# foolwood/SiamMask

Measured on AMD Instinct MI355X. Metric: frames/sec (255x255 search, 127x127 template), higher is better.
Workload: dtype f16

## Files before the change

siammask_amd/_lib.py:

```python
import ctypes
import os
import subprocess

import torch

_HERE = os.path.dirname(os.path.abspath(__file__))
LIB_PATH = os.environ.get("SMK_LIB") or os.path.join(_HERE, "libsiammask_hip.so")
CSRC = os.path.join(_HERE, "csrc")

DTYPE = {"f32": 0, "fp32": 0, "float32": 0, "f16": 1, "fp16": 1, "float16": 1, "half": 1,
         "f16x3": 2}
VARIANT = {"rpn": 0, "base": 1, "sharp": 2}
TRACK_BOX, TRACK_MASK, TRACK_NO_MASK_HEAD = 0, 1, 2

SYMBOLS = (
    "smk_version", "smk_last_error", "smk_create", "smk_destroy", "smk_set_weight",
    "smk_finalize_weights", "smk_template", "smk_track", "smk_refine", "smk_set_decode_params", "smk_decode", "smk_step", "smk_set_graph_mode", "smk_seq_status", "smk_seq_sync_check", "smk_set_result_ring", "smk_result_ring_cursor", "smk_set_pipeline", "smk_pipeline_join", "smk_pipeline_observe",
    "smk_debug_read", "smk_debug_seq_inject", "smk_tune", "smk_tune_get", "smk_profile", "smk_profile_dump", "smk_op_conv2d_ex", "smk_op_conv2d", "smk_op_dw_xcorr",
    "smk_op_maxpool3x3s2", "smk_op_conv_seq", "smk_host_conv2d_ex", "smk_host_plan_conv", "smk_host_plan_seq", "smk_bench_conv", "smk_packed_size", "smk_export_packed",
    "smk_import_packed", "smk_crop_resize", "smk_paste_mask", "smk_paste_labels", "smk_mask_rbox_workspace", "smk_mask_rbox",
    "smk_trk_state_bytes", "smk_trk_set", "smk_trk_plan", "smk_trk_advance", "smk_crop_resize_dev", "smk_paste_mask_dev",
    "smk_host_trk_plan", "smk_host_trk_advance",
)


class ConvGeom(ctypes.Structure):
    _fields_ = [(n, ctypes.c_int) for n in (
        "B", "Cin", "H", "W", "Cout", "k", "stride", "pad", "dil", "relu", "res_mode",
        "win", "ups", "Hl", "Wl", "org_y", "org_x", "pos_mul", "pos_add", "cin_off", "cin_len")]


class SeqOp(ctypes.Structure):
    _fields_ = [("g", ConvGeom), ("src", ctypes.c_int), ("res_src", ctypes.c_int), ("sync", ctypes.c_int),
                ("cfg", ctypes.c_int), ("kstag", ctypes.c_int), ("w_host", ctypes.c_void_p), ("b_host", ctypes.c_void_p),
                ("y_dev", ctypes.c_void_p)]


class TrkCfg(ctypes.Structure):
    _fields_ = [("context_amount", ctypes.c_double), ("lr", ctypes.c_double)] + [(n, ctypes.c_int) for n in (
        "exemplar_size", "instance_size", "total_stride", "base_size", "score_size", "mask_size")]


class SmkError(RuntimeError):
    code = 0


E_SEQ = -6


def build_library(force=False, verbose=False):
    if force:
        subprocess.check_call(["make", "-C", CSRC, "clean"], stdout=subprocess.DEVNULL)
    out = subprocess.run(["make", "-C", CSRC, "-j", "4"], stdout=subprocess.PIPE,
                         stderr=subprocess.STDOUT, universal_newlines=True)
    if verbose or out.returncode != 0:
        print(out.stdout)
    if out.returncode != 0:
        raise SmkError("building libsiammask_hip.so failed")
    return LIB_PATH


_lib = None


def lib():
    global _lib
    if _lib is not None:
        return _lib
    if not os.path.exists(LIB_PATH):
        raise SmkError(
            "%s is missing: the HIP extension has not been built (run `python -c 'import "
            "__graft_entry__ as g; g.build()'` or `make -C siammask_amd/csrc`). There is no "
            "CPU fallback." % LIB_PATH)
    L = ctypes.CDLL(LIB_PATH)
    vp, ci, fp = ctypes.c_void_p, ctypes.c_int, ctypes.c_void_p
    L.smk_version.restype = ci
    L.smk_last_error.restype = ctypes.c_char_p
    L.smk_create.argtypes = [ctypes.POINTER(vp), ci, ci, ci, ci]
    L.smk_destroy.argtypes = [vp]
    L.smk_set_weight.argtypes = [vp, ctypes.c_char_p, fp, ctypes.POINTER(ctypes.c_int64), ci]
    L.smk_finalize_weights.argtypes = [vp]
    L.smk_template.argtypes = [vp, fp, ci, vp]
    L.smk_track.argtypes = [vp, fp, ci, ci, fp, fp, fp, vp]
    L.smk_refine.argtypes = [vp, vp, ci, ci, fp, vp]
    L.smk_set_decode_params.argtypes = [vp, fp, ci, ci, ctypes.c_double, ctypes.c_double]
    L.smk_decode.argtypes = [vp, fp, fp, ci, fp, vp, fp, vp]
    L.smk_step.argtypes = [vp, fp, ci, ci, fp, fp, fp, fp, fp, fp, vp]
    L.smk_set_graph_mode.argtypes = [vp, ci]
    L.smk_debug_seq_inject.argtypes = [vp, ci]
    L.smk_set_result_ring.argtypes = [vp, vp, vp, ci, ci]
    L.smk_set_pipeline.argtypes = [vp, ci]
    L.smk_pipeline_join.argtypes = [vp, vp]
    L.smk_pipeline_observe.argtypes = [vp, vp]
    L.smk_result_ring_cursor.argtypes = [vp, ctypes.POINTER(ci), ci, vp]
    L.smk_seq_sync_check.argtypes = [vp, vp, ctypes.POINTER(ci)]
    L.smk_tune.argtypes = [ctypes.c_char_p, ci]
    L.smk_tune_get.argtypes = [ctypes.c_char_p, ctypes.POINTER(ci)]
    L.smk_profile.argtypes = [vp, ci]
    L.smk_profile_dump.argtypes = [vp, ctypes.c_char_p, ci]
    ip = ctypes.POINTER(ci)
    L.smk_debug_read.argtypes = [vp, ctypes.c_char_p, fp, ip, ip, ip, vp]
    gp = ctypes.POINTER(ConvGeom)
    L.smk_op_conv2d_ex.argtypes = [ci, ci, gp, fp, fp, fp, fp, vp, fp, vp]
    L.smk_op_conv2d.argtypes = [ci, ci, fp, ci, ci, ci, ci, fp, fp, ci, ci, ci, ci, ci, ci, fp, fp, vp]
    L.smk_op_dw_xcorr.argtypes = [ci, fp, fp, ci, ci, ci, ci, ci, ci, fp, vp]
    L.smk_op_maxpool3x3s2.argtypes = [ci, fp, ci, ci, ci, ci, fp, vp]
    L.smk_host_conv2d_ex.argtypes = [gp, fp, fp, fp, fp, vp, fp]
    L.smk_host_plan_conv.argtypes = [gp, ci, ci, ip, ip, ip, ip]
    L.smk_packed_size.argtypes = [vp, ctypes.POINTER(ctypes.c_uint64)]
    L.smk_export_packed.argtypes = [vp, vp, ctypes.c_uint64]
    L.smk_import_packed.argtypes = [vp, vp, ctypes.c_uint64]
    L.smk_crop_resize.argtypes = [vp, ctypes.c_int64, ci, ci, vp, vp, ci, ci, fp, vp]
    L.smk_paste_mask.argtypes = [fp, ci, vp, ci, ci, ci, ctypes.c_float, ctypes.c_float, vp, fp, vp]
    L.smk_paste_labels.argtypes = [fp, ci, vp, ci, ci, ci, ctypes.c_float, ctypes.c_float, vp, vp]
    L.smk_mask_rbox_workspace.argtypes = [ci, ci, ci]
    L.smk_mask_rbox.argtypes = [vp, ci, ci, ci, ctypes.c_double, vp, ctypes.c_size_t, vp, vp]
    cp = ctypes.POINTER(TrkCfg)
    L.smk_trk_state_bytes.argtypes = [ci]
    L.smk_trk_set.argtypes = [vp, ci, vp, vp, vp, ci, ci, vp]
    L.smk_trk_plan.argtypes = [vp, ci, cp, vp]
    L.smk_trk_advance.argtypes = [vp, ci, cp, vp, ci, vp, ci, vp]
    L.smk_host_trk_plan.argtypes = [vp, ci, cp]
    L.smk_host_trk_advance.argtypes = [vp, ci, cp, vp, ci, vp, ci]
    L.smk_crop_resize_dev.argtypes = [vp, ctypes.c_int64, ci, ci, vp, ci, ci, fp, vp]
    L.smk_paste_mask_dev.argtypes = [fp, fp, ci, ci, vp, ci, ci, ci, ci, ctypes.c_float, ctypes.c_float, vp, fp, vp]
    L.smk_op_conv_seq.argtypes = [ctypes.POINTER(SeqOp), ci, fp, ci, ctypes.POINTER(ctypes.c_float), fp, ip, vp]
    L.smk_host_plan_seq.argtypes = [ctypes.POINTER(SeqOp), ci, ci, ip, ip, ip]
    L.smk_bench_conv.argtypes = [ci, ci, gp, ci, ci, ctypes.POINTER(ctypes.c_float), vp]
    for name in SYMBOLS:
        fn = getattr(L, name)
        if name not in ("smk_last_error",):
            fn.restype = ctypes.c_size_t if name in ("smk_mask_rbox_workspace", "smk_trk_state_bytes") else ci
    _lib = L
    for kv in filter(None, os.environ.get("SMK_TUNE", "").split(",")):
        k, v = kv.split("=")
        check(L.smk_tune(k.strip().encode(), int(v)))
    return L


def check(rc):
    if rc != 0:
        msg = lib().smk_last_error()
        e = SmkError("libsiammask_hip error %d: %s" % (rc, msg.decode() if msg else "?"))
        e.code = rc
        raise e


def current_stream_ptr():
    return ctypes.c_void_p(torch.cuda.current_stream().cuda_stream)


def tune(**kw):
    for k, v in kw.items():
        check(lib().smk_tune(k.encode(), int(v)))


def tune_get(key):
    v = ctypes.c_int(0)
    check(lib().smk_tune_get(key.encode(), ctypes.byref(v)))
    return v.value
```

siammask_amd/csrc/conv_igemm.hip:

```cpp
#include <hip/hip_runtime.h>
#include "smk_kernels.h"

namespace smk {

typedef _Float16 half8 __attribute__((ext_vector_type(8)));
typedef _Float16 half4 __attribute__((ext_vector_type(4)));
typedef float floatx16 __attribute__((ext_vector_type(16)));
typedef float floatx4 __attribute__((ext_vector_type(4)));

template <typename T> struct Traits;
template <> struct Traits<float> {
    static constexpr int VE = 4;
    typedef floatx4 frag_t;
    typedef floatx4 out4_t;
    static __device__ inline void mma(floatx16 &acc, const frag_t &a, const frag_t &b) {
        acc = __builtin_amdgcn_mfma_f32_32x32x2f32(a[0], b[0], acc, 0, 0, 0);
        acc = __builtin_amdgcn_mfma_f32_32x32x2f32(a[1], b[1], acc, 0, 0, 0);
        acc = __builtin_amdgcn_mfma_f32_32x32x2f32(a[2], b[2], acc, 0, 0, 0);
        acc = __builtin_amdgcn_mfma_f32_32x32x2f32(a[3], b[3], acc, 0, 0, 0);
    }
    static __device__ inline floatx4 load4(const float *p) { return *(const floatx4 *)p; }
    static __device__ inline void store4(float *p, floatx4 v) { *(floatx4 *)p = v; }
    static constexpr int EV = 4;
    static __device__ inline void loadv(const float *p, float (&v)[4]) {
// ... 760 lines not shown
        for (int q = 0; q < EV; q += 4) {
            const floatx4 b4 = *(const floatx4 *)(bias + n + q);
            bv[q] = b4[0]; bv[q + 1] = b4[1]; bv[q + 2] = b4[2]; bv[q + 3] = b4[3];
        }
        T *out = (T *)p.out;
        const float *ecol = ebase + ((c4 >> 6) * WK) * (64 * LDE) + (c4 & 63);
#pragma unroll
        for (int ps = 0; ps < NPASS; ++ps) {
            const int row = ps * RPP + r0;
            if (row < nvalid) {
                const float *er = ecol + ((row >> 6) * WN * WK) * (64 * LDE) + (row & 63) * LDE;
                float v[EV];
#pragma unroll
                for (int q = 0; q < EV; q += 4) {
                    floatx4 x = *(const floatx4 *)(er + q);
#pragma unroll
                    for (int kq = 1; kq < WK; ++kq) x += *(const floatx4 *)(er + kq * (64 * LDE) + q);
                    v[q] = x[0]; v[q + 1] = x[1]; v[q + 2] = x[2]; v[q + 3] = x[3];
                }
#pragma unroll
                for (int q = 0; q < EV; ++q) {
                    float x = v[q] + bv[q];
                    if (p.res_mode == RES_PRE_RELU) x += rv[ps][q];
                    if (p.relu) x = fmaxf(x, 0.f);
                    if (p.res_mode == RES_POST_RELU) x += rv[ps][q];
                    v[q] = x;
                }
                TR::storev(out + (size_t)(m0 + row) * p.Cos + p.cout_off + n, v);
            }
        }
    }
}

static int halo_patch_rows(const ConvParams &p, int BM) {
    const int howo = p.Ho * p.Wo, Wp = p.Wl + 2 * p.pad;
    const int tpi = (howo + BM - 1) / BM;
    int worst = 0;
    for (int tl = 0; tl < tpi; ++tl) {
        const int ml0 = tl * BM, nv = howo - ml0 < BM ? howo - ml0 : BM;
        const int oy0 = ml0 / p.Wo, ox0 = ml0 % p.Wo, ml = ml0 + nv - 1, oyl = ml / p.Wo, oxl = ml % p.Wo;
        const int rows = oyl * Wp + oxl - (oy0 * Wp + ox0) + 2 * p.dil * Wp + 2 * p.dil + 1;
        if (rows > worst) worst = rows;
    }
    return worst;
}
constexpr int HALO_AROWS_128 = 320, HALO_AROWS_64 = 224;

template <typename T, int WM, int WN, int WK, int AROWS, int NSLOT, int NPATCH>
static int launch_halo_t(const ConvParams &p, hipStream_t s) {
    constexpr int BM = 64 * WM, BN = 64 * WN;
    const int tpi = (p.Ho * p.Wo + BM - 1) / BM;
    if (halo_patch_rows(p, BM) > AROWS) return 1;
    dim3 grid(p.B * tpi * ((p.Nst + BN - 1) / BN));
    hipLaunchKernelGGL((conv3x3_halo_kernel<T, WM, WN, WK, AROWS, NSLOT, NPATCH>), grid, dim3(512), 0, s, p);
    return hipGetLastError() == hipSuccess ? 0 : -4;
}

bool conv_halo_eligible(const ConvParams &p, int dtype, int bm) {
    const int ch = dtype == DT_F16 ? 64 : 32;
    if (p.kh != 3 || p.kw != 3 || p.stride != 1 || p.stride_x != 1 || p.ups || p.groups > 1 || p.Ci % ch != 0 ||
        p.out_mode != OUT_NHWC || !p.buf_lds || p.Wo != p.Wl + 2 * p.pad - 2 * p.dil)
        return false;
    return halo_patch_rows(p, bm == 128 ? 128 : 64) <= (bm == 128 ? HALO_AROWS_128 : HALO_AROWS_64);
}

int launch_conv_halo(const ConvParams &p, int dtype, int bm, void *stream) {
    hipStream_t s = (hipStream_t)stream;
    const int ch = dtype == DT_F16 ? 64 : 32;
    if (!conv_halo_eligible(p, dtype, bm)) return 1;
    const int ch_n = p.Ci / ch;
    const long wgs64 = (long)p.B * ((p.Ho * p.Wo + 63) / 64) * ((p.Nst + 127) / 128);
    const bool db = bm == 64 && g_tune.halo_db && ch_n >= 2 && wgs64 <= 256;
    if (dtype == DT_F16) {
        if (bm == 128) return launch_halo_t<_Float16, 2, 2, 1, HALO_AROWS_128, 2, 1>(p, s);
        return db ? launch_halo_t<_Float16, 1, 2, 2, HALO_AROWS_64, 3, 2>(p, s) : launch_halo_t<_Float16, 1, 2, 2, HALO_AROWS_64, 3, 1>(p, s);
    }
    if (bm == 128) return launch_halo_t<float, 2, 2, 1, HALO_AROWS_128, 2, 1>(p, s);
    return db ? launch_halo_t<float, 1, 2, 2, HALO_AROWS_64, 3, 2>(p, s) : launch_halo_t<float, 1, 2, 2, HALO_AROWS_64, 3, 1>(p, s);
}

}
namespace smk {
#include "refine_chain_body.inc"
constexpr int CM_CONV_LDS = IgemmLds<2, 2, 1, 128, 2>::v;
constexpr int CM_LDS = CMax<RC_LDS, 2 * CM_CONV_LDS>::v;

__global__ __launch_bounds__(1024) void chain_mask_kernel(const RefineChainParams rp, const ConvBatch cb) {
    __shared__ __attribute__((aligned(16))) unsigned char smem[CM_LDS];
    if ((int)blockIdx.x < rp.B) {
        refine_chain_body<false>(rp, (int)blockIdx.x, smem);
    } else {
        const int half = threadIdx.x >> 9;
        const int bx = 2 * ((int)blockIdx.x - rp.B) + half;
        if (bx < cb.start[cb.n])
            conv_igemm_body<_Float16, 2, 2, 1, 128, OUT_NCHW_F32, 2>(cb, bx, 0, half * 512, smem + half * CM_CONV_LDS);
    }
    if (rp.tail_sem) {
        __syncthreads();
        if (threadIdx.x == 0) {
            const unsigned prev = __hip_atomic_fetch_add(rp.tail_sem + 5, 1u, __ATOMIC_RELAXED, __HIP_MEMORY_SCOPE_AGENT);
            if (prev == gridDim.x - 1) {
                __hip_atomic_store(rp.tail_sem + 5, 0u, __ATOMIC_RELAXED, __HIP_MEMORY_SCOPE_AGENT);
                __hip_atomic_fetch_add(rp.tail_sem, 1u, __ATOMIC_RELEASE, __HIP_MEMORY_SCOPE_AGENT);
            }
        }
    }
}

int launch_chain_mask(const RefineChainParams &rp, ConvBatch &cb, void *stream) {
    if (rp.v2_cs != 32 || rp.v1_cs != 16 || rp.v0_cs != 8 || cb.n != 1) return -1;
    ConvParams &p = cb.p[0];
    if (p.out_mode != OUT_NCHW_F32 || p.groups > 1) return -1;
    const int tiles = ((p.M + 127) / 128) * ((p.Nst + 127) / 128);
    if (tiles & 1) return 1;
    cb.start[0] = 0;
    for (int i = 1; i <= CONV_BATCH_MAX; ++i) cb.start[i] = tiles;
    p.ksplit = 1;
    hipLaunchKernelGGL(chain_mask_kernel, dim3(rp.B + (tiles + 1) / 2), dim3(1024), 0, (hipStream_t)stream, rp, cb);
    return hipGetLastError() == hipSuccess ? 0 : -4;
}

template <typename T>
__global__ void conv_naive_kernel(const ConvParams p) {
    typedef Traits<T> TR;
    constexpr int VE = TR::VE;
    const int g = blockIdx.z;
    const int cin_off = p.cin_off + g * p.g_cin_off;
    const T *wgt = (const T *)p.wgt + (size_t)g * p.g_wgt_off * p.Kpad;
    const float *bias = p.bias + g * p.g_wgt_off;
    const int cout_off = p.cout_off + g * p.g_cout_off;
    const int nq = p.Nst / 4;
    const long total = (long)p.M * nq;
    const T *in = (const T *)p.in;
    for (long idx = (long)blockIdx.x * blockDim.x + threadIdx.x; idx < total;
         idx += (long)gridDim.x * blockDim.x) {
        const int m = (int)(idx / nq), n = (int)(idx - (long)m * nq) * 4;
        const RowInfo r = row_info(p, m, p.pos);
        float acc[4] = {0.f, 0.f, 0.f, 0.f};
        for (int kvec = 0; kvec < p.K; kvec += VE) {
            const KDecode d = decode_k(kvec, p.Ci, p.kw);
            const long off = gather_offset(p, r, d, cin_off);
            if (off < 0) continue;
            for (int e = 0; e < VE; ++e) {
                const float a = (float)in[off + e];
                for (int j = 0; j < 4; ++j)
                    acc[j] = fmaf(a, (float)wgt[(size_t)(n + j) * p.Kpad + kvec + e], acc[j]);
            }
        }
        if (p.out_mode == OUT_NHWC) {
            floatx4 v = {acc[0] + bias[n], acc[1] + bias[n + 1], acc[2] + bias[n + 2], acc[3] + bias[n + 3]};
            floatx4 rv = {0.f, 0.f, 0.f, 0.f};
            if (p.res_mode != RES_NONE)
                rv = TR::load4((const T *)p.res + (size_t)m * p.res_Cs + p.res_coff + n);
            if (p.res_mode == RES_PRE_RELU) v += rv;
            if (p.relu)
                for (int j = 0; j < 4; ++j) v[j] = fmaxf(v[j], 0.f);
            if (p.res_mode == RES_POST_RELU) v += rv;
            TR::store4((T *)p.out + (size_t)m * p.Cos + cout_off + n, v);
        } else {
            const int hw = p.Ho * p.Wo;
            const int b = m / hw, pos = m - b * hw;
            for (int j = 0; j < 4; ++j)
                if (n + j < p.N) {
                    float v = acc[j] + bias[n + j];
                    if (p.relu) v = fmaxf(v, 0.f);
                    ((float *)p.out)[((size_t)b * p.N + n + j) * hw + pos] = v;
                }
        }
    }
}

Tuning g_tune;

static int default_kt(int bm, int bn) { return (bm == 64 && bn == 64) ? 256 : 128; }
static int default_stages(int bm, int bn, int kt) {
    if (bm == 128 && bn == 128 && kt == 128) return 2;
    return (bm + bn) * kt * 3 <= 160 * 1024 ? 3 : 2;
}

TileChoice choose_tile(const ConvParams &p, int dtype) {
    (void)dtype;
    TileChoice t;
    if (g_tune.force_tile) {
        static const int tb[6][2] = {{0, 0}, {128, 128}, {128, 64}, {64, 128}, {64, 64}, {256, 128}};
        t.bm = tb[g_tune.force_tile][0];
        t.bn = tb[g_tune.force_tile][1];
        t.stages = default_stages(t.bm, t.bn, default_kt(t.bm, t.bn));
    } else {
        const long ng = p.groups > 0 ? p.groups : 1;
        auto tiles = [&](int bm, int bn) {
            return (long)((p.M + bm - 1) / bm) * ((p.Nst + bn - 1) / bn) * ng * 16 / g_tune.min_blocks_x16;
        };
        if (p.Nst <= 64) {
            if (tiles(128, 64) >= 200) { t.bm = 128; t.bn = 64; t.stages = 3; }
            else { t.bm = 64; t.bn = 64; t.stages = 3; }
        } else if (tiles(256, 128) >= 900 && p.K >= 2048) { t.bm = 256; t.bn = 128; t.stages = 3; }
        else if (tiles(128, 128) >= 300) { t.bm = 128; t.bn = 128; t.stages = 2; }
        else if (tiles(64, 128) >= 200) { t.bm = 64; t.bn = 128; t.stages = 3; }
        else { t.bm = 64; t.bn = 64; t.stages = 3; }
    }
    t.kt = g_tune.kt ? g_tune.kt : default_kt(t.bm, t.bn);
// ... 117 lines not shown
```

siammask_amd/csrc/conv_plan.cpp:

```cpp
#include "conv_plan.h"

#include <algorithm>
#include <cstdio>
#include <cstdlib>
#include <cstring>

using namespace smk;

TileChoice tile_from_code(int code, const ConvParams &p, int dtype) {
    TileChoice t = choose_tile(p, dtype);
    static const int tb[6][2] = {{0, 0}, {128, 128}, {128, 64}, {64, 128}, {64, 64}, {256, 128}};
    const int tile = code & 15, kt = (code >> 4) & 3, st = (code >> 6) & 3;
    if (tile >= 1 && tile <= 5) {
        t.bm = tb[tile][0]; t.bn = tb[tile][1];
        t.kt = (t.bm == 64 && t.bn == 64) ? 256 : 128;
        t.stages = (t.bm == 128 && t.bn == 128) ? 2 : 3;
    }
    if (kt) t.kt = kt == 2 ? 256 : 128;
    if (t.bm == 64 && t.bn == 64) t.kt = 256;
    if (t.bm == 256) t.kt = 128;
    if (st) t.stages = st + 1;
    return t;
}

// ... 252 lines not shown
    return st;
}

double seq_fabric_bytes(const SeqLayer *L, int n, int B, const void *late_read) {
    double ext = 0.0;
    for (int i = 0; i < n; ++i) {
        const SeqLayer &l = L[i];
        bool in_inside = false, res_inside = l.res == nullptr, out_read = false;
        for (int j = 0; j < n; ++j) {
            if (j < i && L[j].out == l.in) in_inside = true;
            if (j < i && l.res && L[j].out == l.res) res_inside = true;
            if (j > i && (L[j].in == l.out || L[j].res == l.out)) out_read = true;
        }
        bool in_counted = false, res_counted = false;
        for (int j = 0; j < i; ++j) {
            if (L[j].in == l.in || L[j].res == l.in) in_counted = true;
            if (l.res && (L[j].in == l.res || L[j].res == l.res)) res_counted = true;
        }
        const double px_in = (double)B * l.Hs * l.Ws, px_out = (double)B * l.Ho * l.Wo;
        ext += (double)l.Nst * l.Kpad * 2.0;
        if (!in_inside && !in_counted) ext += px_in * l.Cs * 2.0;
        if (!res_inside && !res_counted) ext += px_out * l.res_Cs * 2.0;
        if (!out_read || l.out == late_read) ext += px_out * l.Nst * 2.0;
    }
    return ext;
}

const int WREG_TILE[9][2] = {{0, 0}, {64, 256}, {64, 128}, {64, 64}, {128, 256}, {128, 128}, {128, 64}, {96, 256}, {32, 64}};
int wreg_choice(const ConvParams &p, const ConvOpt &o, int dtype, long ncu) {
    if (o.algo_naive || !conv_wreg_eligible(p, dtype)) return 0;
    if (o.wreg) return o.wreg;
    if (g_tune.wreg >= 2) return g_tune.wreg - 1;
    if (!g_tune.wreg) return 0;
    const long K = (long)p.kh * p.kw * p.Ci;
    if (g_tune.wreg_policy == 1) {
        if (p.kh > 3) return 0;
        if (p.kh == 3 && p.stride == 1 && K <= 1152) return 0;
        if (p.M > 16384 && !(p.Nst >= 512 || (K >= 2304 && p.Nst >= 128) || (K >= 1024 && p.Nst >= 256) ||
                             (p.kh == 3 && p.stride == 2)))
            return 0;
        static const int cand[4] = {4, 1, 2, 3};
        const int nr = (p.Nst + 63) / 64 * 64, ng = p.groups > 0 ? p.groups : 1;
        for (int ci = 0; ci < 4; ++ci) {
            const int bm = WREG_TILE[cand[ci]][0], bn = WREG_TILE[cand[ci]][1];
            if (bn > nr && bn > 64) continue;
            if ((long)((p.M + bm - 1) / bm) * ((p.Nst + bn - 1) / bn) * ng >= 150) {
                if (cand[ci] == 4 && g_tune.wreg96) {
                    const long tn = (p.Nst + 255) / 256 * ng;
                    const long t128 = (long)((p.M + 127) / 128) * tn, t96 = (long)((p.M + 95) / 96) * tn;
                    if (((t128 + ncu - 1) / ncu) * 128 > ((t96 + ncu - 1) / ncu) * 96 && t96 <= 4 * ncu) return 7;
                }
                return cand[ci];
            }
        }
        if (g_tune.wreg32 && (long)((p.M + 63) / 64) * ((p.Nst + 63) / 64) * ng < g_tune.wreg32) return 8;
        return 3;
    }
    if (p.M < 4096) return 0;
    if (p.kh == 3 && K >= 2304 && p.Nst >= 512)
        return ((long)((p.M + 127) / 128) * ((p.Nst + 255) / 256) >= 200) ? 4 : 1;
    if (p.M > 16384) return 0;
    if (p.kh == 1 && K >= 512 && p.Nst <= 256) return p.Nst >= 192 ? 2 : 3;
    if (p.kh == 3 && p.stride == 2 && K >= 1152 && p.Nst <= 128) return 3;
    return 0;
}
int wreg_stages(int ctx_dtype, int B) {
    if (g_tune.wreg_stages) return g_tune.wreg_stages;
    return (ctx_dtype == DT_F16X3 || (B >= 1 && B <= 2)) ? 4 : 3;
}
int wreg_stages_from_code(int code) {
    const int st = (code >> 6) & 3;
    return st == 0 ? wreg_stages(DT_F16, 0) : (st == 1 ? 8 : (st == 2 ? 3 : 4));
}

bool pp_choice(const ConvParams &p, const ConvOpt &o, int dtype, long ncu) {
    if (!g_tune.pp || o.algo_naive || o.halo || o.wreg || o.tile_code || !conv_pp_eligible(p, dtype)) return false;
    const long K = (long)p.kh * p.kw * p.Ci;
    const long tiles = (long)((p.M + 255) / 256) * ((p.Nst + 255) / 256);
    const long rounds = (tiles + ncu - 1) / ncu;
    if (tiles < 200 || tiles * 10 < rounds * ncu * 9 || p.Nst < 256 || (p.Nst % 256) != 0) return false;
    return g_tune.pp == 2 || K >= 2304;
}

ConvPlan plan_conv(const ConvParams &p, const ConvOpt &o, const PackedConv &pc, int dtype, int B, long ncu) {
    const int kd = kdtype(dtype);
    ConvPlan pl;
    pl.tile = tile_from_code(o.tile_code, p, kd);
    if (o.algo_naive) { pl.kind = CK_NAIVE; return pl; }
    int bm = halo_choice(pc, p, o, kd);
    if (bm && !o.halo && conv_ksplit(p, kd, pl.tile) > 1) bm = 0;
    if (pp_choice(p, o, kd, ncu)) { pl.kind = CK_PP; return pl; }
    const int wr = (o.halo || (bm && !o.wreg && g_tune.wreg < 2 && g_tune.wreg_policy == 0)) ? 0 : wreg_choice(p, o, kd, ncu);
    if (wr) {
        pl.kind = CK_WREG; pl.wreg = wr; pl.stages = wreg_stages(dtype, B);
    } else if (bm && conv_halo_eligible(p, kd, bm)) {
        pl.kind = CK_HALO; pl.halo_bm = bm;
    }
    return pl;
}

ConvPlan plan_conv_batch(const ConvBatch &cb, const ConvOpt *const o[], int lead, int dtype, int B, long ncu) {
    const int kd = kdtype(dtype);
    ConvPlan pl;
    int wr = wreg_choice(cb.p[lead], *o[lead], kd, ncu);
    for (int i = 0; i < cb.n && wr; ++i)
        if (!wreg_choice(cb.p[i], *o[i], kd, ncu) || (cb.p[i].groups > 1) != (cb.p[0].groups > 1)) wr = 0;
    if (wr) {
        pl.kind = CK_WREG; pl.wreg = wr; pl.stages = wreg_stages(dtype, B);
    } else {
        pl.tile = tile_from_code(o[lead]->tile_code, cb.p[lead], kd);
    }
    return pl;
}

std::string plan_kernel_name(const ConvPlan &pl, int dtype, int out_mode, int merged) {
    const char *dt = dtname(kdtype(dtype));
    char kn[80], mg[16] = "";
    if (merged) snprintf(mg, sizeof(mg), ",merged%d", merged);
    switch (pl.kind) {
    case CK_NAIVE: return "conv_naive";
    case CK_PP: return "conv_pp<f16,256x256>";
    case CK_HALO: snprintf(kn, sizeof(kn), "conv3x3_halo<%s,%dx128>", dt, pl.halo_bm); break;
    case CK_WREG: snprintf(kn, sizeof(kn), "conv_wreg<%s,%dx%d,s%d%s>", dt, WREG_TILE[pl.wreg][0], WREG_TILE[pl.wreg][1], pl.stages, mg); break;
    default:
        snprintf(kn, sizeof(kn), "conv_igemm<%s,%dx%dx%d,s%d,%s%s>", dt, pl.tile.bm, pl.tile.bn, pl.tile.kt, pl.tile.stages,
                 out_mode == OUT_NCHW_F32 ? "nchw" : "nhwc", mg);
    }
    return kn;
}
```

siammask_amd/csrc/conv_plan.h:

```cpp
#pragma once
#include <string>
#include <vector>

#include "smk_kernels.h"

struct Act {
    void *p = nullptr;
    int H = 0, W = 0, C = 0;
};

struct PackedConv {
    void *w = nullptr;
    void *w_halo = nullptr;
    void *w_frag = nullptr;
    void *w_frag_halo = nullptr;
    void *w_frag16 = nullptr;
    float *bias = nullptr;
    int N = 0;
    int rows = 0;
    int group_rows = 0;
    int groups = 1;
    int Ci = 0, k = 1, K = 0, Kpad = 0;
    int kw = 0;
    int alg_k = 0;
    float *oscale = nullptr;
    int x3_ct = 0, x3_nreal = 0;
    bool x3 = false;
};

struct ConvOpt {
    int stride = 1, pad = 0, dil = 1, relu = 0;
    int stride_x = 0;
    const Act *res = nullptr;
    int res_mode = smk::RES_NONE;
    int res_coff = 0;
    int cin_off = 0;
    int cout_off = 0;
    int n_override = 0;
    int groups = 1;
    bool win = false;
    int Hl = 0, Wl = 0, org_y = 0, org_x = 0;
    const int *pos = nullptr;
    int pos_mul = 0, pos_add = 0;
    bool ups = false;
    float *nchw_out = nullptr;
    int algo_naive = 0;
    int tile_code = 0;
    int halo = 0;
    int wreg = 0;
};

inline int kdtype(int dtype) { return dtype == smk::DT_F16X3 ? smk::DT_F16 : dtype; }
inline const char *dtname(int dt) { return dt == smk::DT_F16 ? "f16" : "f32"; }

#pragma GCC visibility push(hidden)

enum ConvKernel { CK_NAIVE, CK_IGEMM, CK_HALO, CK_WREG, CK_PP };
struct ConvPlan {
    int kind = CK_IGEMM;
    smk::TileChoice tile{};
    int halo_bm = 0;
    int wreg = 0;
    int stages = 0;
};

extern const int WREG_TILE[9][2];

smk::TileChoice tile_from_code(int code, const smk::ConvParams &p, int dtype);
int halo_choice(const PackedConv &pc, const smk::ConvParams &p, const ConvOpt &o, int dtype);
int wreg_choice(const smk::ConvParams &p, const ConvOpt &o, int dtype, long ncu);
int wreg_stages(int ctx_dtype, int B);
int wreg_stages_from_code(int code);
bool pp_choice(const smk::ConvParams &p, const ConvOpt &o, int dtype, long ncu);

ConvPlan plan_conv(const smk::ConvParams &p, const ConvOpt &o, const PackedConv &pc, int dtype, int B, long ncu);
ConvPlan plan_conv_batch(const smk::ConvBatch &cb, const ConvOpt *const *o, int lead, int dtype, int B, long ncu);
std::string plan_kernel_name(const ConvPlan &pl, int dtype, int out_mode, int merged = 0);

bool seq_halo_ok(const smk::ConvParams &p, int bm);
bool seq_layer_from(const smk::ConvParams &p, int dtype, smk::SeqLayer &L, int force_halo = 0);
bool seq_pair_fusable(const smk::SeqLayer *L, int i, int *code);
bool seq_pair_fits(const smk::SeqLayer *L, int i, int B, int *code);

struct SeqRec {
    smk::SeqLayer L;
    const void *wstd = nullptr;
    std::string id;
};
struct SeqPlanEnv {
    int B = 0;
    int nslots = 0;
    bool have_xch = false;
};
struct SeqPlanStats { int pairs = 0, triples = 0, resident = 0; };

SeqPlanStats plan_seq(std::vector<SeqRec> &rec, const SeqPlanEnv &env, const char *locked, const std::vector<const void *> &read_after);
double seq_fabric_bytes(const smk::SeqLayer *L, int n, int B, const void *late_read);

#pragma GCC visibility pop
```

siammask_amd/csrc/engine.cpp:

```cpp
#include <hip/hip_runtime_api.h>

#include <cmath>
#include <cstdarg>
#include <tuple>
#include <cstdio>
#include <cstdlib>
#include <cstring>
#include <functional>
#include <map>
#include <set>
#include <memory>
#include <string>
#include <vector>

#include "../../include/siammask_hip.h"
#include "../../include/siammask_hip_test.h"
#include "conv_plan.h"
#include "smk_kernels.h"
#include "tracker_state.h"

using namespace smk;

static thread_local std::string g_err;
static int g_concurrency_default = 0;
// ... 171 lines not shown
    const char *p3_buf = "a";
    bool graph_mode = false;
    hipStream_t cap_stream = nullptr;
    std::map<GraphKey, hipGraphExec_t> graphs;
    std::map<GraphKey, unsigned long long> graph_used;
    unsigned long long graph_tick = 0;

    std::map<std::string, PackedConv> conv;
    std::map<std::string, void *> buf;
    std::map<std::string, size_t> buf_elems;
    std::set<std::string> buf_alias;
    int *pos_dev = nullptr;
    void *dec_scratch = nullptr;
    float *ks_part = nullptr;
    unsigned *ks_cnt = nullptr;
    unsigned *seq_bar = nullptr;
    float *seq_xch = nullptr;
    int *seq_err = nullptr;
    int *seq_err_host = nullptr;
    int *seq_err_hdev = nullptr;
    int seq_fail = 0;
    bool seq_pending = false;
    std::map<GraphKey, bool> graph_has_seq;
    unsigned long long *seq_clk = nullptr, *seq_clk2 = nullptr;
    int seq_grid = 0;
    bool seq_on = false;
    struct SeqList {
        std::vector<SeqRec> rec;
        double flop = 0.0, bytes = 0.0;
        void clear() { rec.clear(); flop = bytes = 0.0; }
    } seq;

    double *ring_box = nullptr;
    void *ring_ref = nullptr;
    int ring_rows = 0;
    int *ring_cursor = nullptr;

    float anchor_w[8] = {104, 88, 64, 40, 32}, anchor_h[8] = {32, 40, 64, 80, 96};
    int anchor_stride = 8;
    double *window_dev = nullptr;
    double penalty_k = 0.04, window_influence = 0.4;

    bool concurrency = true;
    hipStream_t side[2] = {nullptr, nullptr};
    std::vector<hipEvent_t> ev_pool;
    size_t ev_next = 0;

    bool prof = false;
    bool prof_merge = false;
    struct ProfRec { std::string id, kernel; double flop, bytes; hipEvent_t e0, e1; double ext_bytes = 0.0; };
    std::vector<ProfRec> prof_recs;
    std::vector<hipEvent_t> prof_pool;
    size_t prof_pool_next = 0;

    int pipe_depth = 0;
    int parity_now = 0;
    int pipe_parity = 0;
    int last_parity = 0;
    hipStream_t pipe_stream = nullptr;
    std::vector<hipEvent_t> pipe_ev;
    size_t pipe_ev_next = 0;
    bool tail_pending = false;
    hipEvent_t tail_ev = nullptr;
    int ring_batch = 0;
    unsigned *pipe_cnt = nullptr;
    bool tail2_pending = false;
    GraphKey tail2_key, tail2_gated_key;
    int wave_prio_now = 0;
};

struct StepRec {
    bool gate_late = false;
    bool mark_fold = false;
    bool two = false;
    bool seq_exit = false;
    bool tail_fold = false;
    bool defer_mask = false;
    bool ring = false;
    bool ring_refine = false;
    bool seq_exit_done = false;
    bool done_folded = false;
    bool ring_ref_folded = false;
    bool has_seq = false;
    bool mask_join_pending = false;
    struct DeferredMask {
        bool have = false;
        ConvParams p = {};
        double flop = 0.0, bytes = 0.0;
    } deferred_mask;
};

struct ProfScope {
    smk_ctx *c; hipStream_t s; int idx = -1;
    ProfScope(smk_ctx *c_, hipStream_t s_, const std::string &id, const std::string &kernel, double flop,
              double bytes) : c(c_), s(s_) {
        if (!c->prof) return;
        smk_ctx::ProfRec r{id, kernel, flop, bytes, nullptr, nullptr, 0.0};
        if (c->prof_pool_next + 2 > c->prof_pool.size()) return;
        r.e0 = c->prof_pool[c->prof_pool_next++];
        r.e1 = c->prof_pool[c->prof_pool_next++];
        (void)hipEventRecord(r.e0, s);
        c->prof_recs.push_back(r);
        idx = (int)c->prof_recs.size() - 1;
    }
    ~ProfScope() { if (idx >= 0) (void)hipEventRecord(c->prof_recs[idx].e1, s); }
    void ext_bytes(double b) { if (idx >= 0) c->prof_recs[idx].ext_bytes = b; }
    void cancel() { if (idx >= 0 && idx == (int)c->prof_recs.size() - 1) { c->prof_recs.pop_back(); c->prof_pool_next -= 2; } idx = -1; }
};

static int stream_dep(smk_ctx *c, hipStream_t from, hipStream_t to) {
    hipEvent_t e = c->ev_pool[c->ev_next++ % c->ev_pool.size()];
    HIPCHK(hipEventRecord(e, from));
    HIPCHK(hipStreamWaitEvent(to, e, 0));
    return 0;
}
static bool parallel_ok(const smk_ctx *c) { return c->concurrency && !c->prof && c->side[0] && c->side[1]; }

static int nbranch(const smk_ctx *c) { return c->variant == SMK_VARIANT_RPN ? 2 : 3; }

static const HostTensor *find_w(const smk_ctx *c, const std::string &name) {
    auto it = c->host_w.find(name);
    return it == c->host_w.end() ? nullptr : &it->second;
}

static int fold(const smk_ctx *c, const ConvPart &part, int Cout, std::vector<double> &scale,
                std::vector<double> &shift) {
    scale.assign(Cout, 1.0);
    shift.assign(Cout, 0.0);
    if (!part.bn.empty()) {
        const HostTensor *g = find_w(c, part.bn + ".weight"), *b = find_w(c, part.bn + ".bias");
        const HostTensor *m = find_w(c, part.bn + ".running_mean"), *v = find_w(c, part.bn + ".running_var");
        if (!g || !b || !m || !v) return fail(SMK_E_WEIGHT, "missing BatchNorm tensors for %s", part.bn.c_str());
        if ((int)g->data.size() != Cout || (int)b->data.size() != Cout || (int)m->data.size() != Cout ||
            (int)v->data.size() != Cout)
            return fail(SMK_E_WEIGHT, "BatchNorm %s has wrong size", part.bn.c_str());
        for (int i = 0; i < Cout; ++i) {
            const double inv = (double)g->data[i] / std::sqrt((double)v->data[i] + 1e-5);
            scale[i] = inv;
            shift[i] = (double)b->data[i] - (double)m->data[i] * inv;
        }
    }
    if (!part.bias.empty()) {
        const HostTensor *b = find_w(c, part.bias);
        if (!b || (int)b->data.size() != Cout) return fail(SMK_E_WEIGHT, "missing/mis-sized %s", part.bias.c_str());
        for (int i = 0; i < Cout; ++i) shift[i] += (double)b->data[i];
    }
    return 0;
}

static void split_rows_x3(std::vector<float> &rows, int nrows, int Kpad1, int Kpad3, int taps, int Ci0, std::vector<float> &oscale) {
    std::vector<float> out((size_t)nrows * Kpad3, 0.f);
    oscale.assign(nrows, 1.f);
    for (int n = 0; n < nrows; ++n) {
        float mx = 0.f;
        for (int k = 0; k < taps * Ci0; ++k) mx = std::max(mx, std::fabs(rows[(size_t)n * Kpad1 + k]));
        int e = 0;
        if (mx > 0.f) {
            e = 13 - (int)std::floor(std::log2(mx));
            e = std::max(-8, std::min(e, 40));
        }
        const float sc = std::ldexp(1.f, e);
        oscale[n] = std::ldexp(1.f, -e);
        for (int t = 0; t < taps; ++t)
            for (int ci = 0; ci < Ci0; ++ci) {
                const float v = rows[(size_t)n * Kpad1 + (size_t)t * Ci0 + ci] * sc;
                const float hi = (float)(_Float16)v, lo = (float)(_Float16)(v - hi);
                float *d = out.data() + (size_t)n * Kpad3 + (size_t)t * 3 * Ci0 + ci;
                d[0] = hi; d[Ci0] = lo; d[2 * Ci0] = hi;
            }
// ... 477 lines not shown
        snprintf(idn, sizeof(idn), "seq[%s..%s]", r[0].id.c_str(), r[a.n - 1].id.c_str());
        const double fr = (double)a.n / (double)n;
        ProfScope ps(c, s, idn, "conv_seq", c->seq.flop * fr, c->seq.bytes * fr);
        ps.ext_bytes(seq_fabric_bytes(a.L, a.n, B, buf("p2")));
        if (launch_conv_seq(a, c->seq_grid, s))
            return fail(SMK_E_HIP, "launch of %s failed: %s", idn, hipGetErrorString(hipGetLastError()));
        c->seq_pending = rec.has_seq = true;
        if (want_clk) {
            unsigned long long h[2 * SEQ_MAX + 1], h2[(12 + 32) * SEQ_MAX];
            HIPCHK(hipStreamSynchronize(s));
            HIPCHK(hipMemcpy(h, c->seq_clk, sizeof(h), hipMemcpyDeviceToHost));
            if (want_clk2) HIPCHK(hipMemcpy(h2, c->seq_clk2, sizeof(h2), hipMemcpyDeviceToHost));
            seq_print_clk(a, r, idn, h, want_clk2 ? h2 : nullptr);
        }
    }
    c->seq.clear();
    return 0;
}

static int seq_health(smk_ctx *c) {
    if (!c->seq_err_host) return 0;
    const int e = *(volatile int *)c->seq_err_host;
    if (!e) return 0;
    (void)hipDeviceSynchronize();
    c->seq_fail = e;
    if (e != 3) c->seq_grid = 0;
    else c->pipe_depth = 0;
    if (c->pipe_cnt) {
        const unsigned init[16] = {1u, 0u};
        (void)hipMemcpy(c->pipe_cnt, init, sizeof(init), hipMemcpyHostToDevice);
    }
    *(volatile int *)c->seq_err_host = 0;
    (void)hipMemset(c->seq_err, 0, sizeof(int));
    (void)hipMemset(c->seq_bar, 0, 8 * 32 * sizeof(unsigned));
    for (auto &kv : c->graphs) hipGraphExecDestroy(kv.second);
    c->graphs.clear();
    c->graph_used.clear();
    c->graph_has_seq.clear();
    c->seq_pending = false;
    c->tail_pending = false;
    c->tail2_pending = false;
    c->template_B = 0;
    c->track_B = 0;
    if (e == 3)
        return fail(SMK_E_SEQ, "conv_seq_kernel reported: (pipelined step) a gate waited 0.2 s (a tail's gate: 5 s) for its partner on the other stream -- something serialises "
                    "the two queues of this context (a profiler collecting counters does); the results of the calls enqueued on this context "
                    "since then are invalid (the cached template included) and frame steps are serial from here on: call template() again and "
                    "re-submit the frame");
    return fail(SMK_E_SEQ, "conv_seq_kernel reported %s: the results of the calls enqueued on this context since then are invalid "
                "(the cached template included); persistent sequences are now off for this context (per-layer kernels from here "
                "on): call template() again and re-submit the frame",
                e == 1 ? "an uneven distribution of workgroups over the XCDs" : "a team-barrier time-out (another kernel held CUs "
                "for more than 0.2 s, or a second persistent kernel ran beside it)");
}

static bool seq_wanted(const smk_ctx *c, int B) {
    if (!g_tune.seq || c->seq_grid <= 0 || c->dtype != DT_F16) return false;
    if (B >= g_tune.seq_min_batch && B <= g_tune.seq_max_batch) return true;
    if (B == g_tune.seq_extra_batch) return true;
    return B % 8 == 0 && B <= g_tune.seq_mult_max;
}

static void conv_work(const PackedConv &pc, const ConvParams &p, int B, int dtype, double &flop, double &bytes) {
    const int ng = p.groups > 0 ? p.groups : 1;
    const double kreal = pc.alg_k ? (double)pc.alg_k : (double)p.kh * p.kw * p.Ci;
    const size_t es = esize(kdtype(dtype));
    flop += 2.0 * p.M * (double)p.N * kreal * ng;
    bytes += (double)B * (p.ups ? p.Hs * p.Ws : (double)p.Hl * p.Wl) * p.Ci * es * ng + (double)p.M * p.N * ng * (p.out_mode == OUT_NCHW_F32 ? 4 : es) +
             (double)p.N * kreal * es * ng + (p.res ? (double)p.M * p.N * es : 0.0);
}

static int launch_plan(const ConvPlan &pl, ConvBatch &cb, const void *w_halo, int dtype, hipStream_t s, const char *what) {
    int rc;
    switch (pl.kind) {
    case CK_PP: rc = launch_conv_pp(cb.p[0], s); break;
    case CK_WREG: rc = launch_conv_wreg_batch(cb, WREG_TILE[pl.wreg][0], WREG_TILE[pl.wreg][1], pl.stages, s); break;
    case CK_HALO: {
        ConvParams ph = cb.p[0];
        ph.wgt = w_halo;
        rc = launch_conv_halo(ph, dtype, pl.halo_bm, s);
        break;
    }
    case CK_NAIVE: rc = launch_conv_naive(cb.p[0], dtype, s); break;
    default: rc = launch_conv_mfma_batch(cb, dtype, pl.tile, s);
    }
    if (rc == 1) return fail(SMK_E_STATE, "internal: %s is not eligible for the kernel planned for it", what);
    if (rc) return fail(SMK_E_HIP, "launch of %s failed: %s", what, hipGetErrorString(hipGetLastError()));
    return 0;
}

static int run_conv(smk_ctx *c, const char *id, const Act &in, const Act *out, int B, const ConvOpt &o,
                    hipStream_t s, StepRec *rec = nullptr) {
    auto it = c->conv.find(id);
    if (it == c->conv.end()) return fail(SMK_E_STATE, "internal: conv %s not packed", id);
    ConvBatch cb;
    cb.n = 1;
    ConvParams &p = cb.p[0];
    CHK(conv_params(conv_env(c), it->second, in, out, B, o, p));
    double flop = 0.0, bytes = 0.0;
    conv_work(it->second, p, B, c->dtype, flop, bytes);
    if (c->seq_on) {
        SeqLayer L;
        if (!o.algo_naive && !o.halo && !o.wreg && !o.tile_code && seq_layer_from(p, kdtype(c->dtype), L)) {
            c->seq.rec.push_back({L, p.wgt_frag, id});
            c->seq.flop += flop;
            c->seq.bytes += bytes;
            return 0;
        }
        if (!rec) return fail(SMK_E_STATE, "internal: conv %s recorded into a sequence without a step record", id);
        CHK(seq_flush(c, *rec, B, s));
    }
    const ConvPlan pl = plan_conv(p, o, it->second, c->dtype, B, c->ncu);
    ProfScope ps(c, s, id, plan_kernel_name(pl, c->dtype, p.out_mode), flop, bytes);
    char what[80];
    snprintf(what, sizeof(what), "conv %s", id);
    return launch_plan(pl, cb, it->second.w_halo, kdtype(c->dtype), s, what);
}

struct ConvJob { const char *id; const Act *in; const Act *out; ConvOpt o; };

static int run_conv_jobs(smk_ctx *c, const std::vector<ConvJob> &jobs, int B, int lead, hipStream_t s, StepRec *rec = nullptr) {
    if (jobs.empty() || (int)jobs.size() > CONV_BATCH_MAX) return fail(SMK_E_ARG, "internal: bad conv job count");
    if (c->seq_on) {
        const size_t n0 = c->seq.rec.size();
        for (auto &j : jobs) CHK(run_conv(c, j.id, *j.in, j.out, B, j.o, s, rec));
        if (c->seq.rec.size() == n0 + jobs.size())
            for (size_t i = n0; i + 1 < c->seq.rec.size(); ++i) c->seq.rec[i].L.sync = 0;
        return 0;
    }
    ConvBatch cb;
    cb.n = (int)jobs.size();
    bool split_for_halo = g_tune.halo != 0;
    int n_halo = 0;
    for (int i = 0; i < cb.n; ++i) {
        auto it = c->conv.find(jobs[i].id);
        if (it == c->conv.end()) return fail(SMK_E_STATE, "internal: conv %s not packed", jobs[i].id);
        CHK(conv_params(conv_env(c), it->second, *jobs[i].in, jobs[i].out, B, jobs[i].o, cb.p[i]));
        const int bm = halo_choice(it->second, cb.p[i], jobs[i].o, kdtype(c->dtype));
        if (bm) ++n_halo;
        if (bm == 64 || (bm == 0 && cb.p[i].kh == 3)) split_for_halo = false;
    }
    const bool merge_ok = g_tune.merge && (g_tune.merge == 2 || B <= g_tune.merge_max_batch);
    if ((c->prof && !c->prof_merge) || cb.n == 1 || !merge_ok || (split_for_halo && n_halo)) {
        for (auto &j : jobs) CHK(run_conv(c, j.id, *j.in, j.out, B, j.o, s));
        return 0;
    }
    double mflop = 0.0, mbytes = 0.0;
    std::string mid;
    const ConvOpt *opts[CONV_BATCH_MAX];
    for (int i = 0; i < cb.n; ++i) {
        opts[i] = &jobs[i].o;
        if (!c->prof) continue;
        conv_work(c->conv.find(jobs[i].id)->second, cb.p[i], B, c->dtype, mflop, mbytes);
        mid += (i ? "+" : "") + std::string(jobs[i].id);
    }
    const ConvPlan pl = plan_conv_batch(cb, opts, lead, c->dtype, B, c->ncu);
    ProfScope ps(c, s, mid.c_str(), plan_kernel_name(pl, c->dtype, cb.p[lead].out_mode, cb.n), mflop, mbytes);
    char what[80];
    snprintf(what, sizeof(what), "merged conv %s..", jobs[0].id);
    return launch_plan(pl, cb, nullptr, kdtype(c->dtype), s, what);
}

static int run_conv_pair(smk_ctx *c, const char *id3, const Act &in3, const Act &out3, const ConvOpt &o3, const char *id1,
                         const Act &out1, const ConvOpt &o1, int B, hipStream_t s) {
    if (c->dtype != DT_F16 || !g_tune.pair_launch || c->seq_on || parallel_ok(c) || (c->prof && !c->prof_merge)) return 1;
    if (g_tune.pair_launch == 1 && B < 3) return 1;
// ... 137 lines not shown
            if (b == 0) {
                Act r = act(c, RN[st], so, so, X(planes * 4));
                ConvOpt od;
                if (st == 0) { od.stride = 1; od.pad = 0; }
                else if (st == 1) { od.stride = 2; od.pad = 0; }
                else { od.stride = 1; od.pad = 1; }
                if (par) {
                    hipStream_t sd = c->side[0];
                    CHK(stream_dep(c, s, sd));
                    CHK(run_conv(c, id_ds.c_str(), cur, &r, B, od, sd, &rec));
                    CHK(run_conv(c, id_c1.c_str(), cur, &t1, B, o1, s, &rec));
                } else {
                    CHK(run_conv_jobs(c, {{id_ds.c_str(), &cur, &r, od}, {id_c1.c_str(), &cur, &t1, o1}}, B, 0, s, &rec));
                }
                res = r;
            } else if (!c1_done) {
                CHK(run_conv(c, id_c1.c_str(), cur, &t1, B, o1, s, &rec));
            }
            c1_done = false;
            CHK(run_conv(c, (id + "c2").c_str(), t1, &t2, B, o2, s, &rec));
            if (b == 0 && par) CHK(stream_dep(c, c->side[0], s));
            const bool last = b == STAGE_BLOCKS[st] - 1;
            const char *oname = last ? (st == 0 ? "p1" : st == 1 ? "p2" : AN[2]) : ((b & 1) ? BN[st] : AN[st]);
            if (last && st == 2 && cur.p == c->buf.at(AN[2])) oname = BN[2];
            Act out = act(c, oname, so, so, X(planes * 4));
            if (last && st == 2) c->p3_buf = oname;
            ConvOpt o3; o3.relu = 1; o3.res = &res; o3.res_mode = RES_PRE_RELU;
            int paired = 1;
            if (!c->seq_on && st >= 1) {
                if (!last) {
                    char idn[32];
                    snprintf(idn, sizeof(idn), "l%d.%d.c1", st + 1, b + 1);
                    Act t1n = act(c, T1N[st], so, so, X(planes));
                    ConvOpt o1n; o1n.relu = 1;
                    paired = run_conv_pair(c, (id + "c3").c_str(), t2, out, o3, idn, t1n, o1n, B, s);
                    if (paired < 0) return paired;
                    if (paired == 0) c1_done = true;
                } else if (st == 2 && so >= 20) {
                    Act se = act(c, "search", so, so, X(256));
                    ConvOpt oa0;
                    paired = run_conv_pair(c, (id + "c3").c_str(), t2, out, o3, "adjust", se, oa0, B, s);
                    if (paired < 0) return paired;
                    if (paired == 0) adjust_done = true;
                }
            }
            if (paired == 1) CHK(run_conv(c, (id + "c3").c_str(), t2, &out, B, o3, s, &rec));
            cur = out;
            sp = so;
        }
    }
    ConvOpt oa;
    if (sp < 20) {
        Act zf = act(c, "zf", sp - 8, sp - 8, X(256));
        oa.win = true; oa.Hl = oa.Wl = sp - 8; oa.org_y = oa.org_x = 4;
        CHK(run_conv(c, "adjust", cur, &zf, B, oa, s, &rec));
    } else if (!adjust_done) {
        Act se = act(c, "search", sp, sp, X(256));
        CHK(run_conv(c, "adjust", cur, &se, B, oa, s, &rec));
    }
    if (c->seq_on && search_nb > 0 && sp >= 20 && g_tune.seq_search && c->seq.rec.size() < (size_t)SEQ_MAX) {
        Act se = act(c, "search", sp, sp, X(256));
        Act xs = act(c, "xs", sp - 2, sp - 2, X(256 * search_nbt));
        ConvOpt o; o.relu = 1; o.n_override = 256 * search_nb;
        CHK(run_conv(c, "conv_search", se, &xs, B, o, s, &rec));
        if (search_done) *search_done = true;
    }
    if (c->seq_on) CHK(seq_flush(c, rec, B, s));
    c->last_B = B; c->last_S = S;
    return 0;
}

static int seq_template(smk_ctx *c, StepRec &rec, const float *z, int B, hipStream_t s) {
    auto X = [c](int C) { return c->dtype == DT_F16X3 ? X3_PLANES * C : C; };
    CHK(run_backbone(c, rec, z, B, 127, s));
    const int nb = nbranch(c);
    Act zf = act(c, "zf", 7, 7, X(256));
    Act zk = act(c, "zk", 5, 5, X(256 * nb));
    ConvOpt o; o.relu = 1;
    CHK(run_conv(c, "conv_kernel", zf, &zk, B, o, s));
    return 0;
}

static int seq_track(smk_ctx *c, StepRec &rec, const float *x, int B, int flags, float *cls, float *loc, float *mask,
                     hipStream_t s, bool defer_mask_join = false, int phase = PH_ALL) {
    auto X = [c](int C) { return c->dtype == DT_F16X3 ? X3_PLANES * C : C; };
    const bool x3 = c->dtype == DT_F16X3;
    const int nbt = nbranch(c);
    const int nb = (flags & SMK_TRACK_MASK) ? nbt : 2;
    bool search_done = false;
    CHK(run_backbone(c, rec, x, B, 255, s, phase, nb, nbt, &search_done));
    Act se = act(c, "search", 31, 31, X(256));
    Act xs = act(c, "xs", 29, 29, X(256 * nbt));
    ConvOpt o; o.relu = 1; o.n_override = 256 * nb;
    if (!search_done) CHK(run_conv(c, "conv_search", se, &xs, B, o, s));
    if (rec.gate_late) {
        if (launch_pipe_gate(c->pipe_cnt, c->seq_err, c->seq_err_hdev, s, 0, nullptr, c->pipe_cnt + 8)) return fail(SMK_E_HIP, "pipe_gate launch failed");
        rec.has_seq = true;
    }
    Act corr = act(c, "corr", 25, 25, X(256 * nbt));
    Act h0 = act(c, "head0", 25, 25, X(256 * nbt));
    const bool par = parallel_ok(c);
    const bool want_mask = (flags & SMK_TRACK_MASK) && !(flags & SMK_TRACK_NO_MASK_HEAD);
    hipStream_t s_loc = par ? c->side[0] : s, s_cls = (par && want_mask) ? c->side[1] : s;
    bool fused_heads = false;
    if (c->dtype == DT_F16 && g_tune.corr_head && !par) {
        auto ih = c->conv.find("head0"), ic = c->conv.find("cls3"), il = c->conv.find("loc3");
        if (ih != c->conv.end() && ic != c->conv.end() && il != c->conv.end() && ih->second.w_frag && ic->second.w_frag && il->second.w_frag &&
            ih->second.Kpad == 256 && ic->second.Kpad == 256 && il->second.Kpad == 256 && ih->second.group_rows == 256 &&
            ic->second.N == 10 && il->second.N == 20) {
            CorrHeadParams hp;
            memset(&hp, 0, sizeof(hp));
            hp.xs = (const _Float16 *)xs.p; hp.zk = (const _Float16 *)c->buf.at("zk"); hp.corr = (_Float16 *)corr.p; hp.h0 = (_Float16 *)h0.p;
            hp.w0_frag = ih->second.w_frag; hp.b0 = ih->second.bias; hp.w0_bytes = (unsigned)((size_t)ih->second.rows * ih->second.Kpad * 2);
            hp.w3_frag[0] = ic->second.w_frag; hp.b3[0] = ic->second.bias; hp.out3[0] = cls; hp.n3[0] = 10;
            hp.w3_frag[1] = il->second.w_frag; hp.b3[1] = il->second.bias; hp.out3[1] = loc; hp.n3[1] = 20;
            hp.w3_bytes[0] = (unsigned)((size_t)ic->second.rows * ic->second.Kpad * 2);
            hp.w3_bytes[1] = (unsigned)((size_t)il->second.rows * il->second.Kpad * 2);
            hp.B = B; hp.nb = nb; hp.Cs = 256 * nbt;
            const double flop = 2.0 * B * nb * 256.0 * 625 * 25 + 2.0 * B * nb * 625.0 * 256 * 256 + 2.0 * B * 625.0 * 256 * 30;
            const double bytes = (double)B * nb * 256.0 * (29 * 29 + 25 + 2 * 625) * 2 + 3.0 * 256 * 256 * 2 + (double)B * 30 * 625 * 4;
            ProfScope ps(c, s, "dw_xcorr+head0+cls3+loc3", "corr_head", flop, bytes);
            if (launch_corr_head(hp, s)) return fail(SMK_E_HIP, "corr_head launch failed: %s", hipGetErrorString(hipGetLastError()));
            fused_heads = true;
        }
    }
    if (!fused_heads) {
    XcorrParams xp{xs.p, c->buf.at("zk"), corr.p, B, 29, 29, 5, 5, 25, 25, 256 * nb, 256 * nbt};
    {
        const double xb = (double)B * nb * 256.0 * (29 * 29 + 25 + 625) * esize(c->dtype);
        ProfScope ps(c, s, "dw_xcorr", x3 ? "dw_xcorr_x3" : "dw_xcorr", 2.0 * B * nb * 256.0 * 625 * 25, x3 ? (double)X3_PLANES * xb : xb);
        if (x3 ? launch_xcorr_x3(xp, s) : launch_xcorr(xp, kdtype(c->dtype), s)) return fail(SMK_E_HIP, "xcorr launch failed");
    }
    ConvOpt oh; oh.relu = 1; oh.groups = nb;
    CHK(run_conv(c, "head0", corr, &h0, B, oh, s));
    if (par) { CHK(stream_dep(c, s, s_loc)); if (s_cls != s) CHK(stream_dep(c, s, s_cls)); }
    ConvOpt oc; oc.nchw_out = cls; oc.cin_off = 0;
    ConvOpt ol; ol.nchw_out = loc; ol.cin_off = x3 ? X3_PLANES * 256 : 256;
    if (par) {
        CHK(run_conv(c, "cls3", h0, nullptr, B, oc, s_cls));
        CHK(run_conv(c, "loc3", h0, nullptr, B, ol, s_loc));
    } else {
        CHK(run_conv_jobs(c, {{"cls3", &h0, nullptr, oc}, {"loc3", &h0, nullptr, ol}}, B, 1, s));
    }
    }
    if (want_mask) {
        ConvOpt om; om.nchw_out = mask; om.cin_off = x3 ? 2 * X3_PLANES * 256 : 512;
        if (rec.defer_mask && !par) {
            auto it = c->conv.find("mask3");
            if (it == c->conv.end()) return fail(SMK_E_STATE, "internal: conv mask3 not packed");
            CHK(conv_params(conv_env(c), it->second, h0, nullptr, B, om, rec.deferred_mask.p));
            const ConvParams &mp = rec.deferred_mask.p;
            rec.deferred_mask.flop = 2.0 * mp.M * (double)mp.N * mp.kh * mp.kw * mp.Ci;
            rec.deferred_mask.bytes = (double)mp.M * mp.Ci * esize(c->dtype) + (double)mp.M * mp.N * 4 + (double)mp.N * mp.Ci * esize(c->dtype);
            rec.deferred_mask.have = true;
        } else if (defer_mask_join && !par && !c->prof && g_tune.mask_overlap && c->side[0]) {
            CHK(stream_dep(c, s, c->side[0]));
            CHK(run_conv(c, "mask3", h0, nullptr, B, om, c->side[0]));
            rec.mask_join_pending = true;
        } else {
            CHK(run_conv(c, "mask3", h0, nullptr, B, om, s));
        }
    }
    if (par) { CHK(stream_dep(c, s_loc, s)); if (s_cls != s) CHK(stream_dep(c, s_cls, s)); }
    c->last_nb = nb;
    return 0;
}

static bool refine_splittable(const smk_ctx *c, int B) {
    return kdtype(c->dtype) == DT_F16 && g_tune.chain && !parallel_ok(c) && g_tune.merge && (g_tune.merge == 2 || B <= g_tune.merge_max_batch);
}
static int seq_refine(smk_ctx *c, StepRec &rec, int B, float *out, hipStream_t s, int part = 0) {
    const int *pos = c->pos_dev;
    auto X = [c](int C) { return c->dtype == DT_F16X3 ? X3_PLANES * C : C; };
    Act corr = act(c, "corr", 25, 25, X(256 * 3));
    Act p0 = act(c, "p0", 125, 125, X(64)), p1 = act(c, "p1", 63, 63, X(256)), p2 = act(c, "p2", 31, 31, X(512));
    ConvOpt r3; r3.pad = 1; r3.relu = 1;
    ConvOpt w2 = r3; w2.win = true; w2.Hl = w2.Wl = 15; w2.pos = pos; w2.pos_mul = 1; w2.pos_add = -4;
    ConvOpt w1 = r3; w1.win = true; w1.Hl = w1.Wl = 31; w1.pos = pos; w1.pos_mul = 2; w1.pos_add = -8;
    ConvOpt w0 = r3; w0.win = true; w0.Hl = w0.Wl = 61; w0.pos = pos; w0.pos_mul = 4; w0.pos_add = -16;
    const bool par = parallel_ok(c);
    hipEvent_t ev_v2 = nullptr, ev_v1 = nullptr, ev_v0 = nullptr;
    if (par) {
        hipStream_t sd = c->side[0];
        CHK(stream_dep(c, s, sd));
        Act v2a_ = act(c, "rf_v2a", 15, 15, 128), v1a_ = act(c, "rf_v1a", 31, 31, 64), v0a_ = act(c, "rf_v0a", 61, 61, 16);
        CHK(run_conv(c, "v2.0", p2, &v2a_, B, w2, sd));
        ev_v2 = c->ev_pool[c->ev_next++ % c->ev_pool.size()];
        HIPCHK(hipEventRecord(ev_v2, sd));
        CHK(run_conv(c, "v1.0", p1, &v1a_, B, w1, sd));
        ev_v1 = c->ev_pool[c->ev_next++ % c->ev_pool.size()];
        HIPCHK(hipEventRecord(ev_v1, sd));
        CHK(run_conv(c, "v0.0", p0, &v0a_, B, w0, sd));
        ev_v0 = c->ev_pool[c->ev_next++ % c->ev_pool.size()];
        HIPCHK(hipEventRecord(ev_v0, sd));
    }
    Act d1 = act(c, "rf_d", 1, 1, 15 * 15 * 32);
    ConvOpt od; od.win = true; od.Hl = od.Wl = 1; od.pos = pos; od.pos_mul = 1; od.cin_off = c->dtype == DT_F16X3 ? 2 * X3_PLANES * 256 : 512;
    Act v2a = act(c, "rf_v2a", 15, 15, 128), v1a = act(c, "rf_v1a", 31, 31, 64), v0a = act(c, "rf_v0a", 61, 61, 16);
    const bool merged = !par && (!c->prof || c->prof_merge) && g_tune.merge && (g_tune.merge == 2 || B <= g_tune.merge_max_batch);
    if (merged && part != 2) {
        w2.tile_code = 4;
        if (g_tune.rf_wreg & 1) w2.wreg = w1.wreg = w0.wreg = od.wreg = ((g_tune.rf_wreg >> 4) & 15) ? ((g_tune.rf_wreg >> 4) & 15) : 3;
        CHK(run_conv_jobs(c, {{"v2.0", &p2, &v2a, w2}, {"v1.0", &p1, &v1a, w1}, {"v0.0", &p0, &v0a, w0},
                              {"deconv", &corr, &d1, od}}, B, 0, s));
    } else if (part != 2) {
        CHK(run_conv(c, "deconv", corr, &d1, B, od, s));
    }
    Act d = act(c, "rf_d", 15, 15, 32);
    if (kdtype(c->dtype) == DT_F16 && g_tune.chain && !par) {
        if (!merged && part != 2) {
            CHK(run_conv(c, "v2.0", p2, &v2a, B, w2, s));
            CHK(run_conv(c, "v1.0", p1, &v1a, B, w1, s));
            CHK(run_conv(c, "v0.0", p0, &v0a, B, w0, s));
        }
        Act V2 = act(c, "rf_s2", 15, 15, 32), V1 = act(c, "rf_s1", 31, 31, 16), V0 = act(c, "rf_s0", 61, 61, 8);
        ConvOpt r3l = r3;
        r3l.tile_code = g_tune.rf_tile2;
        ConvOpt r3w = r3;
        if ((g_tune.rf_wreg & 2) && merged) r3l.wreg = r3w.wreg = ((g_tune.rf_wreg >> 8) & 15) ? ((g_tune.rf_wreg >> 8) & 15) : 3;
        if (part != 2) CHK(run_conv_jobs(c, {{"v2.2", &v2a, &V2, r3l}, {"v1.2", &v1a, &V1, r3w}, {"v0.2", &v0a, &V0, r3w}}, B, 0, s));
        if (part == 1) return 0;
        static const char *ids[9] = {"h2.0", "h2.2", "post0", "h1.0", "h1.2", "post1", "h0.0", "h0.2", "post2"};
        static const int geo[9][3] = {{225, 32, 32}, {225, 32, 32}, {961, 32, 16}, {961, 16, 16}, {961, 16, 16},
                                      {3721, 16, 4}, {3721, 4, 4}, {3721, 4, 4}, {16129, 4, 1}};
        RefineChainParams rp;
        double flop = 0.0, wbytes = 0.0;
        for (int i = 0; i < 9; ++i) {
            auto it = c->conv.find(ids[i]);
            if (it == c->conv.end()) return fail(SMK_E_STATE, "internal: conv %s not packed", ids[i]);
            const PackedConv &pc = it->second;
            if (pc.k != 3 || pc.groups != 1 || pc.Ci < geo[i][1] || pc.N != geo[i][2])
                return fail(SMK_E_STATE, "internal: conv %s does not have the Refine geometry", ids[i]);
            rp.L[i] = RefineChainLayer{pc.w, pc.bias, pc.Kpad, pc.Ci};
            flop += 2.0 * B * geo[i][0] * 9.0 * geo[i][1] * geo[i][2];
            wbytes += 2.0 * 9.0 * geo[i][1] * geo[i][2];
        }
        rp.d = d.p;
        rp.v2 = V2.p; rp.v1 = V1.p; rp.v0 = V0.p;
        rp.v2_cs = V2.C; rp.v1_cs = V1.C; rp.v0_cs = V0.C;
        rp.out = out;
        rp.B = B;
        rp.clk = nullptr;
        rp.ring = nullptr; rp.ring_cursor = nullptr; rp.ring_done = nullptr; rp.ring_rows = 0;
        rp.tail_sem = nullptr;
        if (rec.ring && c->ring_ref) {
            rp.ring = (_Float16 *)c->ring_ref; rp.ring_cursor = c->ring_cursor; rp.ring_done = (unsigned *)(c->ring_cursor + 1);
            rp.ring_rows = c->ring_rows;
            rec.ring_ref_folded = true;
        }
        static const bool want_clk = getenv("SMK_CHAIN_CLK") != nullptr;
        static unsigned long long *clk_dev = nullptr;
        hipStreamCaptureStatus cst = hipStreamCaptureStatusNone;
        if (want_clk && hipStreamIsCapturing(s, &cst) == hipSuccess && cst == hipStreamCaptureStatusNone) {
            if (!clk_dev) HIPCHK(hipMalloc((void **)&clk_dev, 32 * sizeof(unsigned long long)));
            rp.clk = clk_dev;
        }
        const double cbytes = B * (2.0 * (7200 + 225 * 32 + 961 * 16 + 3721 * 4) + 4.0 * 16129) + wbytes;
        if (rec.deferred_mask.have && !rp.clk) {
            ConvBatch cb;
            cb.n = 1;
            cb.p[0] = rec.deferred_mask.p;
            ProfScope ps(c, s, "refine_chain+mask3", "chain_mask", flop + rec.deferred_mask.flop, cbytes + rec.deferred_mask.bytes);
            if (rec.tail_fold) rp.tail_sem = c->pipe_cnt;
            const int rc = launch_chain_mask(rp, cb, s);
            rp.tail_sem = nullptr;
            if (rc == 0) {
                rec.deferred_mask.have = false;
                if (rec.tail_fold) rec.done_folded = true;
                return 0;
            }
            if (rc != 1) return fail(SMK_E_HIP, "chain_mask launch failed: %s", hipGetErrorString(hipGetLastError()));
            ps.cancel();
        }
        ProfScope ps(c, s, "refine_chain", "refine_chain", flop, cbytes);
        if (launch_refine_chain(rp, s)) return fail(SMK_E_HIP, "refine_chain launch failed: %s", hipGetErrorString(hipGetLastError()));
        if (rp.clk) {
            unsigned long long hh[22];
            HIPCHK(hipStreamSynchronize(s));
            HIPCHK(hipMemcpy(hh, clk_dev, sizeof(hh), hipMemcpyDeviceToHost));
            {
                const unsigned long long *h = hh;
                fprintf(stderr, "refine_chain layers (us): load=%.2f", (double)(h[1] - h[0]) * 0.01);
                for (int i = 0; i < 9; ++i) fprintf(stderr, " %s=%.2f", ids[i], (double)(h[i + 2] - h[i + 1]) * 0.01);
                fprintf(stderr, " total=%.2f\n", (double)(h[10] - h[0]) * 0.01);
            }
        }
        return 0;
    }
    Act h2a = act(c, "rf_h2a", 15, 15, 32), h2b = act(c, "rf_h2b", 15, 15, 32);
    CHK(run_conv(c, "h2.0", d, &h2a, B, r3, s));
    CHK(run_conv(c, "h2.2", h2a, &h2b, B, r3, s));
    Act s2 = act(c, "rf_s2", 15, 15, 32);
    if (par) CHK(hipStreamWaitEvent(s, ev_v2, 0) == hipSuccess ? 0 : fail(SMK_E_HIP, "wait ev_v2"));
    else if (!merged) CHK(run_conv(c, "v2.0", p2, &v2a, B, w2, s));
    ConvOpt a2 = r3; a2.res = &h2b; a2.res_mode = RES_POST_RELU;
    CHK(run_conv(c, "v2.2", v2a, &s2, B, a2, s));
    Act u0 = act(c, "rf_u0", 31, 31, 16);
    ConvOpt pu0; pu0.pad = 1; pu0.ups = true; pu0.Hl = pu0.Wl = 31;
    CHK(run_conv(c, "post0", s2, &u0, B, pu0, s));
    Act h1a = act(c, "rf_h1a", 31, 31, 16), h1b = act(c, "rf_h1b", 31, 31, 16);
    CHK(run_conv(c, "h1.0", u0, &h1a, B, r3, s));
    CHK(run_conv(c, "h1.2", h1a, &h1b, B, r3, s));
    Act s1 = act(c, "rf_s1", 31, 31, 16);
    if (par) CHK(hipStreamWaitEvent(s, ev_v1, 0) == hipSuccess ? 0 : fail(SMK_E_HIP, "wait ev_v1"));
    else if (!merged) CHK(run_conv(c, "v1.0", p1, &v1a, B, w1, s));
    ConvOpt a1 = r3; a1.res = &h1b; a1.res_mode = RES_POST_RELU;
    CHK(run_conv(c, "v1.2", v1a, &s1, B, a1, s));
    Act u1 = act(c, "rf_u1", 61, 61, 8);
    ConvOpt pu1; pu1.pad = 1; pu1.ups = true; pu1.Hl = pu1.Wl = 61;
    CHK(run_conv(c, "post1", s1, &u1, B, pu1, s));
    Act h0a = act(c, "rf_h0a", 61, 61, 8), h0b = act(c, "rf_h0b", 61, 61, 8);
    CHK(run_conv(c, "h0.0", u1, &h0a, B, r3, s));
    CHK(run_conv(c, "h0.2", h0a, &h0b, B, r3, s));
    Act s0 = act(c, "rf_s0", 61, 61, 8);
    if (par) CHK(hipStreamWaitEvent(s, ev_v0, 0) == hipSuccess ? 0 : fail(SMK_E_HIP, "wait ev_v0"));
    else if (!merged) CHK(run_conv(c, "v0.0", p0, &v0a, B, w0, s));
    ConvOpt a0 = r3; a0.res = &h0b; a0.res_mode = RES_POST_RELU;
    CHK(run_conv(c, "v0.2", v0a, &s0, B, a0, s));
    ConvOpt pu2; pu2.pad = 1; pu2.ups = true; pu2.Hl = pu2.Wl = 127; pu2.nchw_out = out;
    CHK(run_conv(c, "post2", s0, nullptr, B, pu2, s));
    return 0;
}

template <typename F>
static int capture_graph(smk_ctx *c, const GraphKey &key, const StepRec &rec, F &&body) {
    if (!c->cap_stream) HIPCHK(hipStreamCreateWithFlags(&c->cap_stream, hipStreamNonBlocking));
    HIPCHK(hipStreamBeginCapture(c->cap_stream, hipStreamCaptureModeThreadLocal));
    const bool pend0 = c->seq_pending;
    int rc = body(c->cap_stream);
    c->seq_pending = pend0;
    hipGraph_t g = nullptr;
    hipError_t e = hipStreamEndCapture(c->cap_stream, &g);
    if (rc) { if (g) hipGraphDestroy(g); return rc; }
    if (e != hipSuccess) return fail(SMK_E_HIP, "hipStreamEndCapture: %s", hipGetErrorString(e));
    hipGraphExec_t ex = nullptr;
    e = hipGraphInstantiate(&ex, g, nullptr, nullptr, 0);
    hipGraphDestroy(g);
    if (e != hipSuccess) return fail(SMK_E_HIP, "hipGraphInstantiate: %s", hipGetErrorString(e));
    while (c->graphs.size() >= 64) {
        auto lru = c->graph_used.begin();
        for (auto u = c->graph_used.begin(); u != c->graph_used.end(); ++u)
            if (u->second < lru->second) lru = u;
        auto g = c->graphs.find(lru->first);
        if (g != c->graphs.end()) { hipGraphExecDestroy(g->second); c->graphs.erase(g); }
        c->graph_has_seq.erase(lru->first);
        c->graph_used.erase(lru);
    }
// ... 346 lines not shown
    HIPCHK(hipSetDevice(c->device));
    CHK(seq_health(c));
    hipStream_t s = (hipStream_t)stream;
    CHK(pipe_join(c, s, true));
    c->parity_now = c->last_parity = 0;
    GraphKey key{0, B, 0, {z}};
    StepRec rec;
    int rc = run_maybe_graph(c, key, s, rec, [&](hipStream_t st) { return seq_template(c, rec, z, B, st); });
    if (rc) return rc;
    c->template_B = B;
    c->track_B = 0;
    return 0;
}

int smk_track(smk_ctx *c, const float *x, int B, int flags, float *cls, float *loc, float *mask, void *stream) {
    if (!c || !x || !cls || !loc) return fail(SMK_E_ARG, "smk_track: null argument");
    if (!c->finalized) return fail(SMK_E_STATE, "smk_track: weights not finalized");
    if (c->template_B == 0) return fail(SMK_E_STATE, "smk_track: smk_template has not been called");
    if (B != c->template_B)
        return fail(SMK_E_ARG, "smk_track: batch %d != template batch %d (models/rpn.py:33 requires equality)", B,
                    c->template_B);
    if ((flags & SMK_TRACK_MASK) && c->variant == SMK_VARIANT_RPN)
        return fail(SMK_E_ARG, "smk_track: the rpn variant has no mask branch");
    if ((flags & SMK_TRACK_MASK) && !(flags & SMK_TRACK_NO_MASK_HEAD) && !mask)
        return fail(SMK_E_ARG, "smk_track: mask_out is NULL");
    HIPCHK(hipSetDevice(c->device));
    CHK(seq_health(c));
    hipStream_t s = (hipStream_t)stream;
    CHK(pipe_join(c, s, true));
    c->parity_now = c->last_parity = 0;
    GraphKey key{1, B, flags, {x, cls, loc, mask}};
    StepRec rec;
    int rc = run_maybe_graph(c, key, s, rec, [&](hipStream_t st) { return seq_track(c, rec, x, B, flags, cls, loc, mask, st); });
    if (rc) return rc;
    c->track_B = (flags & SMK_TRACK_MASK) ? B : 0;
    return 0;
}

int smk_refine(smk_ctx *c, const int32_t *pos, int on_device, int B, float *out, void *stream) {
    if (!c || !pos || !out) return fail(SMK_E_ARG, "smk_refine: null argument");
    if (c->variant != SMK_VARIANT_SHARP) return fail(SMK_E_ARG, "smk_refine: only the sharp variant has a Refine module");
    if (c->track_B == 0) return fail(SMK_E_STATE, "smk_refine: needs a preceding smk_track with SMK_TRACK_MASK");
    if (B != c->track_B) return fail(SMK_E_ARG, "smk_refine: batch %d != tracked batch %d", B, c->track_B);
    HIPCHK(hipSetDevice(c->device));
    CHK(seq_health(c));
    hipStream_t s = (hipStream_t)stream;
    CHK(pipe_join(c, s, true));
    c->parity_now = c->last_parity;
    if (!on_device) {
        for (int i = 0; i < 2 * B; ++i)
            if (pos[i] < 0 || pos[i] >= 25) return fail(SMK_E_ARG, "smk_refine: pos[%d]=%d outside [0,25)", i, pos[i]);
        HIPCHK(hipMemcpyAsync(c->pos_dev, pos, sizeof(int) * 2 * B, hipMemcpyHostToDevice, s));
    } else {
        HIPCHK(hipMemcpyAsync(c->pos_dev, pos, sizeof(int) * 2 * B, hipMemcpyDeviceToDevice, s));
    }
    GraphKey key{2, B, c->parity_now, {out}};
    StepRec rec;
    return run_maybe_graph(c, key, s, rec, [&](hipStream_t st) { return seq_refine(c, rec, B, out, st); });
}

enum { KNOB_RAW = 0, KNOB_BOOL = -1 };
struct Knob { const char *name; int *slot; const char *accept; int conv; const char *product; };
#ifdef SMK_MEASURE
static int g_measure_build = 1;
#else
static int g_measure_build = 0;
#endif
static const Knob KNOBS[] = {
    {"xcd_mode", &g_tune.xcd_mode, "*", KNOB_RAW, nullptr},
    {"force_tile", &g_tune.force_tile, "0..5", KNOB_RAW, nullptr},
    {"min_blocks_x16", &g_tune.min_blocks_x16, "*", KNOB_RAW, nullptr},
    {"concurrency", &g_concurrency_default, "*", KNOB_RAW, nullptr},
    {"stages", &g_tune.stages, "0|2..4", KNOB_RAW, nullptr},
    {"kt", &g_tune.kt, "0|128|256", KNOB_RAW, nullptr},
    {"prio", &g_tune.prio, "-1..3", KNOB_RAW, nullptr},
    {"nt_store", &g_tune.nt_store, "*", KNOB_BOOL, nullptr},
    {"merge", &g_tune.merge, "0..2", KNOB_RAW, nullptr},
    {"merge_max_batch", &g_tune.merge_max_batch, "*", KNOB_RAW, nullptr},
    {"rf_wreg", &g_tune.rf_wreg, "*", KNOB_RAW, nullptr},
    {"rf_tile2", &g_tune.rf_tile2, "0..5", KNOB_RAW, nullptr},
    {"nchw_tn_major", &g_tune.nchw_tn_major, "*", KNOB_BOOL, nullptr},
    {"chain", &g_tune.chain, "*", KNOB_BOOL, nullptr},
    {"chain_mask", &g_tune.chain_mask, "*", KNOB_BOOL, nullptr},
    {"corr_head", &g_tune.corr_head, "*", KNOB_BOOL, nullptr},
    {"pair_launch", &g_tune.pair_launch, "0..3", KNOB_RAW, nullptr},
    {"halo", &g_tune.halo, "0|1|64|128", KNOB_RAW, nullptr},
    {"halo_db", &g_tune.halo_db, "*", KNOB_BOOL, nullptr},
    {"ksplit", &g_tune.ksplit, "0|1|2|4", KNOB_RAW, nullptr},
    {"xc_ch", &g_tune.xc_ch, "32|64", KNOB_RAW, nullptr},
    {"xc_full", &g_tune.xc_full, "0..2", KNOB_RAW, nullptr},
    {"stem_fused", &g_tune.stem_fused, "*", KNOB_BOOL, nullptr},
    {"l1_fused", &g_tune.l1_fused, "*", KNOB_BOOL, nullptr},
    {"buf_lds", &g_tune.buf_lds, "*", KNOB_BOOL, nullptr},
    {"a_stage", &g_tune.a_stage, "*", KNOB_BOOL, nullptr},
    {"mask_overlap", &g_tune.mask_overlap, "*", KNOB_BOOL, nullptr},
    {"wreg", &g_tune.wreg, "0..7", KNOB_RAW, nullptr},
    {"wreg_policy", &g_tune.wreg_policy, "0|1", KNOB_RAW, nullptr},
    {"wreg_stages", &g_tune.wreg_stages, "0|3..8", KNOB_RAW, "0|3|4"},
    {"wreg96", &g_tune.wreg96, "*", KNOB_BOOL, nullptr},
    {"wreg32", &g_tune.wreg32, "0..4096", KNOB_RAW, nullptr},
    {"npw", &g_tune.npw, "2|4", KNOB_RAW, nullptr},
    {"res_nt", &g_tune.res_nt, "*", KNOB_BOOL, nullptr},
    {"pp", &g_tune.pp, "0..2", KNOB_RAW, nullptr},
    {"x3_fused", &g_tune.x3_fused, "*", KNOB_BOOL, nullptr},
    {"ablate", &g_tune.ablate, "*", 127, "0"},
    {"front_occ1", &g_tune.front_occ1, "*", 3, "0"},
    {"seq", &g_tune.seq, "*", KNOB_BOOL, nullptr},
    {"seq_spoll", &g_tune.seq_spoll, "*", KNOB_BOOL, nullptr},
    {"seq_kstag", &g_tune.seq_kstag, "0..2", KNOB_RAW, nullptr},
    {"seq_kstag_mask", &g_tune.seq_kstag_mask, "*", 7, nullptr},
    {"seq_tall", &g_tune.seq_tall, "0..2", KNOB_RAW, nullptr},
    {"seq_fuse", &g_tune.seq_fuse, "0..3", KNOB_RAW, nullptr},
    {"seq_fuse3", &g_tune.seq_fuse3, "0..2", KNOB_RAW, "0"},
    {"seq_pair2d", &g_tune.seq_pair2d, "0..2", KNOB_RAW, "0"},
    {"seq_deep", &g_tune.seq_deep, "*", KNOB_BOOL, "0"},
    {"seq_ds128", &g_tune.seq_ds128, "*", KNOB_BOOL, nullptr},
    {"seq_halo", &g_tune.seq_halo, "*", KNOB_BOOL, nullptr},
    {"seq_yres", &g_tune.seq_yres, "*", KNOB_BOOL, nullptr},
    {"seq_search", &g_tune.seq_search, "*", KNOB_BOOL, nullptr},
    {"seq_first_stage", &g_tune.seq_first_stage, "0..3", KNOB_RAW, "1..3"},
    {"seq_min_batch", &g_tune.seq_min_batch, ">=1", KNOB_RAW, nullptr},
    {"seq_max_batch", &g_tune.seq_max_batch, ">=1", KNOB_RAW, nullptr},
    {"seq_extra_batch", &g_tune.seq_extra_batch, "*", KNOB_RAW, nullptr},
    {"seq_mult_max", &g_tune.seq_mult_max, ">=0", KNOB_RAW, nullptr},
    {"main_prio", &g_tune.main_prio, "0..3", KNOB_RAW, nullptr},
    {"pipe_late", &g_tune.pipe_late, "*", KNOB_BOOL, nullptr},
    {"seq_fused_last", &g_seq_last.pairs, nullptr, KNOB_RAW, nullptr},
    {"seq_yres_last", &g_seq_last.resident, nullptr, KNOB_RAW, nullptr},
    {"seq_fused3_last", &g_seq_last.triples, nullptr, KNOB_RAW, nullptr},
    {"measure_build", &g_measure_build, nullptr, KNOB_RAW, nullptr},
};

static bool knob_accepts(const char *spec, int v) {
    if (!strcmp(spec, "*")) return true;
    for (const char *t = spec; t; t = strchr(t, '|') ? strchr(t, '|') + 1 : nullptr) {
        if (t[0] == '>' && t[1] == '=') {
            if (v >= atoi(t + 2)) return true;
            continue;
        }
        char *e = nullptr;
        const long lo = strtol(t, &e, 10), hi = (e[0] == '.' && e[1] == '.') ? strtol(e + 2, nullptr, 10) : lo;
        if (v >= lo && v <= hi) return true;
    }
    return false;
}

static const Knob *find_knob(const char *key) {
    for (const Knob &k : KNOBS)
        if (!strcmp(key, k.name)) return &k;
    return nullptr;
}

int smk_tune(const char *key, int value) {
    if (!key) return fail(SMK_E_ARG, "smk_tune: key is NULL");
    const Knob *k = find_knob(key);
    if (!k) return fail(SMK_E_ARG, "smk_tune: unknown key %s", key);
    if (!k->accept) return fail(SMK_E_ARG, "smk_tune: %s is a read-only diagnostic", key);
    if (!knob_accepts(k->accept, value)) return fail(SMK_E_ARG, "smk_tune: %s takes %s, not %d", key, k->accept, value);
#ifndef SMK_MEASURE
    if (k->product && !knob_accepts(k->product, value))
        return fail(SMK_E_ARG, "smk_tune: %s %d is a measured alternative, only in a library built with `make MEASURE=1` (this one takes %s)",
                    key, value, k->product);
#endif
    if (k->slot == &g_tune.rf_wreg && (((value >> 4) & 15) > 8 || ((value >> 8) & 15) > 8))
        return fail(SMK_E_ARG, "smk_tune: rf_wreg tile codes (bits 4..7, 8..11) 0..8");
    *k->slot = k->conv == KNOB_BOOL ? value != 0 : (k->conv > 0 ? value & k->conv : value);
    return 0;
}

int smk_tune_get(const char *key, int *value) {
    if (!key || !value) return fail(SMK_E_ARG, "smk_tune_get: null argument");
    const Knob *k = find_knob(key);
    if (!k) return fail(SMK_E_ARG, "smk_tune_get: unknown key %s", key);
    *value = *k->slot;
    return 0;
}

int smk_profile(smk_ctx *c, int enable) {
// ... 31 lines not shown
    for (size_t i = 0; i < order.size(); ++i) {
        char line[512];
        const Agg &a = order[i].second;
        snprintf(line, sizeof(line), "%s{\"id\":\"%s\",\"kernel\":\"%s\",\"calls\":%d,\"ms\":%.6f,\"flop\":%.6e,\"bytes\":%.6e,\"ext_bytes\":%.6e}",
                 i ? "," : "", order[i].first.c_str(), a.kernel.c_str(), a.calls, a.ms, a.flop, a.bytes, a.ext);
        js += line;
    }
    js += "]";
    if ((int)js.size() + 1 > cap) return fail(SMK_E_ARG, "smk_profile_dump: buffer too small (%zu needed)", js.size() + 1);
    memcpy(buf, js.c_str(), js.size() + 1);
    return 0;
}

static void fill_decode_params(smk_ctx *c, const float *cls, const float *loc, int B, const double *target_wh, int *pos_out,
                               double *box_out, DecodeParams &p) {
    memset(&p, 0, sizeof(p));
    p.cls = cls; p.loc = loc; p.target_wh = target_wh; p.window = c->window_dev;
    p.pos_out = pos_out; p.box_out = box_out;
    {
        char *q = (char *)c->dec_scratch;
        p.part_val = (double *)q;             q += (size_t)c->maxB * 8 * 8;
        p.part_box = (double *)q;             q += (size_t)c->maxB * 64 * 8;
        p.part_idx = (int *)q;                q += (size_t)c->maxB * 8 * 4;
        p.arrived = (unsigned *)q;
    }
    p.B = B; p.A = 5; p.S = 25; p.stride = c->anchor_stride;
    for (int i = 0; i < 5; ++i) { p.anchor_w[i] = c->anchor_w[i]; p.anchor_h[i] = c->anchor_h[i]; }
    p.penalty_k = c->penalty_k; p.window_influence = c->window_influence;
}

static int seq_decode(smk_ctx *c, const StepRec &rec, const float *cls, const float *loc, int B, const double *target_wh, int *pos_out,
                      double *box_out, hipStream_t s) {
    DecodeParams p;
    fill_decode_params(c, cls, loc, B, target_wh, pos_out, box_out, p);
    if (rec.ring && c->ring_box && box_out) {
        p.ring_box = c->ring_box; p.ring_cursor = c->ring_cursor; p.ring_done = (unsigned *)(c->ring_cursor + 1);
        p.ring_rows = c->ring_rows; p.ring_advance = 1;
        if (rec.ring_refine) {
            p.ring_cursor = c->ring_cursor + 2; p.ring_done = (unsigned *)(c->ring_cursor + 3);
        } else {
            p.ring_also = c->ring_cursor + 2;
        }
    }
    if (rec.mark_fold) { p.mark = c->pipe_cnt + 2; p.mark_arrived = c->pipe_cnt + 4; }
    ProfScope ps(c, s, "decode", "decode", 0.0, (double)B * 30 * 625 * 4);
    if (launch_decode(p, s)) return fail(SMK_E_HIP, "decode launch failed");
    return 0;
}

int smk_set_decode_params(smk_ctx *c, const float *anchor_wh, int n_anchor, int stride, double penalty_k,
                          double window_influence) {
    if (!c) return fail(SMK_E_ARG, "ctx is NULL");
    if (anchor_wh) {
        if (n_anchor != 5) return fail(SMK_E_ARG, "smk_set_decode_params: kernels are specialised for 5 anchors");
        for (int i = 0; i < 5; ++i) { c->anchor_w[i] = anchor_wh[2 * i]; c->anchor_h[i] = anchor_wh[2 * i + 1]; }
    }
    if (stride > 0) c->anchor_stride = stride;
    c->penalty_k = penalty_k;
    c->window_influence = window_influence;
    CHK(pipe_quiesce(c));
    for (auto &kv : c->graphs) hipGraphExecDestroy(kv.second);
    c->graphs.clear();
    c->graph_used.clear();
    return 0;
}

int smk_decode(smk_ctx *c, const float *cls, const float *loc, int B, const double *target_wh, int32_t *pos_out,
               double *box_out, void *stream) {
    if (!c || !cls || !loc || !target_wh) return fail(SMK_E_ARG, "smk_decode: null argument");
    if (B < 1 || B > c->maxB) return fail(SMK_E_ARG, "smk_decode: batch %d not in [1,%d]", B, c->maxB);
    HIPCHK(hipSetDevice(c->device));
    CHK(pipe_join(c, (hipStream_t)stream, true));
    return seq_decode(c, StepRec(), cls, loc, B, target_wh, pos_out ? pos_out : c->pos_dev, box_out, (hipStream_t)stream);
}

static StepRec step_rec(const smk_ctx *c, const float *refine_out) {
    StepRec rec;
    rec.ring = c->ring_rows > 0;
    rec.ring_refine = refine_out != nullptr && c->ring_ref != nullptr;
    return rec;
}

static int step_track_decode(smk_ctx *c, StepRec &rec, const float *x, int B, int flags, const double *target_wh, float *cls, float *loc,
                             float *mask, double *box_out, float *refine_out, hipStream_t st, bool defer_mask_join, int phase) {
    rec.defer_mask = refine_out && mask && (flags & SMK_TRACK_MASK) && !(flags & SMK_TRACK_NO_MASK_HEAD) &&
                     kdtype(c->dtype) == DT_F16 && g_tune.chain && g_tune.chain_mask && !parallel_ok(c) &&
                     (B <= 16 ||
                      rec.two);
    CHK(seq_track(c, rec, x, B, flags, cls, loc, mask, st, defer_mask_join, phase));
    return seq_decode(c, rec, cls, loc, B, target_wh, c->pos_dev, box_out, st);
}

static int step_tail(smk_ctx *c, StepRec &rec, int B, float *mask, double *box_out, float *refine_out, hipStream_t st, int part = 0) {
    auto mask3 = [&]() {
        rec.deferred_mask.have = false;
        Act h0 = act(c, "head0", 25, 25, 256 * nbranch(c));
        ConvOpt om; om.nchw_out = mask; om.cin_off = 512;
        return run_conv(c, "mask3", h0, nullptr, B, om, st);
    };
    if (part == 1 && rec.deferred_mask.have) CHK(mask3());
    if (refine_out) CHK(seq_refine(c, rec, B, refine_out, st, part));
    if (part == 1) return 0;
    if (rec.deferred_mask.have) CHK(mask3());
    if (rec.mask_join_pending) CHK(stream_dep(c, c->side[0], st));
    if (c->ring_rows > 0 && refine_out && c->ring_ref && !rec.ring_ref_folded) {
        RingParams rg{box_out, refine_out, nullptr, (_Float16 *)c->ring_ref, c->ring_cursor,
                      (unsigned *)(c->ring_cursor + 1), c->ring_rows, B, 127 * 127};
        ProfScope ps(c, st, "ring_commit", "ring_commit", 0.0, (double)B * (64.0 * 2 + (refine_out ? 127.0 * 127 * 6 : 0.0)));
        if (launch_ring_commit(rg, st)) return fail(SMK_E_HIP, "ring_commit launch failed: %s", hipGetErrorString(hipGetLastError()));
    }
    return 0;
}

static int step_pipelined_enqueue(smk_ctx *c, const float *x, int B, int flags, const double *target_wh, float *cls, float *loc,
                                  float *mask, double *box_out, float *refine_out, hipStream_t s) {
    const int par = c->pipe_parity;
    c->parity_now = par;
    int64_t pk, wi;
    memcpy(&pk, &c->penalty_k, 8); memcpy(&wi, &c->window_influence, 8);
    const std::vector<const void *> io{x, target_wh, cls, loc, mask, box_out, refine_out, (const void *)pk, (const void *)wi};
    const bool graphs = c->graph_mode;
    const bool late = g_tune.pipe_late && !(seq_wanted(c, B) && !parallel_ok(c));
    const bool two = c->pipe_depth >= 2 && graphs && !late && refine_splittable(c, B);
    const int fl = flags | (par << 16) | (late ? 1 << 17 : 0) | (two ? 1 << 18 : 0);
    const GraphKey km{11, B, fl, io}, kt{12, B, fl, io}, kt2g{13, B, fl, io}, kt2n{14, B, fl, io};
    auto main_ = [&](hipStream_t st, StepRec &rec) {
        struct PrioScope { smk_ctx *c; PrioScope(smk_ctx *c_) : c(c_) { c->wave_prio_now = g_tune.main_prio; } ~PrioScope() { c->wave_prio_now = 0; } } prio_scope(c);
        CHK(run_backbone(c, rec, x, B, 255, st, PH_FRONT));
        if (!late) {
            if (launch_pipe_gate(c->pipe_cnt, c->seq_err, c->seq_err_hdev, st, 0, nullptr, c->pipe_cnt + 8)) return fail(SMK_E_HIP, "pipe_gate launch failed");
            rec.has_seq = true;
        }
        rec.gate_late = late;
        rec.mark_fold = true;
        rec.two = two;
        rec.seq_exit = two;
        CHK(step_track_decode(c, rec, x, B, flags, target_wh, cls, loc, mask, box_out, refine_out, st, false, PH_BACK));
        if (two && !rec.seq_exit_done && launch_pipe_done(c->pipe_cnt + 7, st)) return fail(SMK_E_HIP, "pipe_done launch failed");
        return 0;
    };
    auto tail = [&](hipStream_t st, StepRec &rec, int part, bool gated) {
        if (gated && launch_pipe_gate(c->pipe_cnt + (part == 2 ? 7 : 2), c->seq_err, c->seq_err_hdev, st, 1, part == 2 ? nullptr : c->pipe_cnt + 8)) return fail(SMK_E_HIP, "pipe_gate launch failed");
        rec.tail_fold = part == 0;
        CHK(step_tail(c, rec, B, mask, box_out, refine_out, st, part));
        if (part != 2 && !rec.done_folded && launch_pipe_done(c->pipe_cnt, st)) return fail(SMK_E_HIP, "pipe_done launch failed");
        return 0;
    };
    const StepRec tail_rec = step_rec(c, refine_out);
    StepRec main_rec = tail_rec;
    bool have = c->graphs.count(km) && c->graphs.count(kt);
    if (two) have = have && c->graphs.count(kt2g) && c->graphs.count(kt2n);
    if (graphs && !have) {
        drop_graph(c, km); drop_graph(c, kt); drop_graph(c, kt2g); drop_graph(c, kt2n);
        CHK(capture_graph(c, km, main_rec, [&](hipStream_t st) { return main_(st, main_rec); }));
        StepRec t = tail_rec;
        t.deferred_mask = main_rec.deferred_mask;
        CHK(capture_graph(c, kt, t, [&](hipStream_t st) { return tail(st, t, two ? 1 : 0, true); }));
        if (two) {
            StepRec t2g = tail_rec, t2n = tail_rec;
            CHK(capture_graph(c, kt2g, t2g, [&](hipStream_t st) { return tail(st, t2g, 2, true); }));
            CHK(capture_graph(c, kt2n, t2n, [&](hipStream_t st) { return tail(st, t2n, 2, false); }));
        }
        bool ok = c->graphs.count(km) && c->graphs.count(kt);
        if (two) ok = ok && c->graphs.count(kt2g) && c->graphs.count(kt2n);
        if (!ok) return fail(SMK_E_STATE, "internal: pipelined step graphs evicted while capturing");
    }
    if (!two && c->tail2_pending) CHK(pipe_flush(c));
    CHK(graphs ? launch_graph(c, km, s) : main_(s, main_rec));
    if (!graphs) c->seq_pending = true;
    c->tail_pending = false;
    if (two) {
        if (c->tail2_pending) CHK(launch_graph(c, c->tail2_gated_key, c->pipe_stream));
        else if (launch_pipe_gate(c->pipe_cnt + 7, c->seq_err, c->seq_err_hdev, c->pipe_stream, 1)) return fail(SMK_E_HIP, "pipe_gate launch failed");
        CHK(launch_graph(c, kt, c->pipe_stream));
        c->tail2_pending = true;
        c->tail2_key = kt2n;
        c->tail2_gated_key = kt2g;
    } else if (graphs) CHK(launch_graph(c, kt, c->pipe_stream));
    else {
        StepRec t = tail_rec;
        t.deferred_mask = main_rec.deferred_mask;
        CHK(tail(c->pipe_stream, t, 0, true));
    }
    hipEvent_t e_tail = c->pipe_ev[c->pipe_ev_next++ % c->pipe_ev.size()];
    HIPCHK(hipEventRecord(e_tail, c->pipe_stream));
    c->tail_ev = e_tail;
    c->tail_pending = true;
    c->last_parity = par;
    c->pipe_parity = par ^ 1;
    return 0;
}
static int step_pipelined(smk_ctx *c, const float *x, int B, int flags, const double *target_wh, float *cls, float *loc,
                          float *mask, double *box_out, float *refine_out, hipStream_t s) {
    const int rc = step_pipelined_enqueue(c, x, B, flags, target_wh, cls, loc, mask, box_out, refine_out, s);
    if (rc) {
        (void)hipDeviceSynchronize();
        (void)pipe_reset_counters(c);
        c->tail_pending = false;
    }
    return rc;
}

int smk_step(smk_ctx *c, const float *x, int B, int flags, const double *target_wh, float *cls, float *loc,
             float *mask, double *box_out, float *refine_out, void *stream) {
    if (!c || !x || !cls || !loc || !target_wh || !box_out) return fail(SMK_E_ARG, "smk_step: null argument");
    if (!c->finalized) return fail(SMK_E_STATE, "smk_step: weights not finalized");
    if (c->template_B == 0) return fail(SMK_E_STATE, "smk_step: smk_template has not been called");
    if (B != c->template_B) return fail(SMK_E_ARG, "smk_step: batch %d != template batch %d", B, c->template_B);
    if (refine_out && (c->variant != SMK_VARIANT_SHARP || !(flags & SMK_TRACK_MASK)))
        return fail(SMK_E_ARG, "smk_step: refine needs the sharp variant and SMK_TRACK_MASK");
    if ((flags & SMK_TRACK_MASK) && c->variant == SMK_VARIANT_RPN) return fail(SMK_E_ARG, "smk_step: rpn has no mask branch");
    if ((flags & SMK_TRACK_MASK) && !(flags & SMK_TRACK_NO_MASK_HEAD) && !mask) return fail(SMK_E_ARG, "smk_step: mask_out is NULL");
    if (c->ring_rows > 0 && B != c->ring_batch)
        return fail(SMK_E_ARG, "smk_step: batch %d, but the result ring was set for batch %d (smk_set_result_ring)", B, c->ring_batch);
    HIPCHK(hipSetDevice(c->device));
    CHK(seq_health(c));
    hipStream_t s = (hipStream_t)stream;
    if (c->pipe_depth > 0 && refine_out && !c->prof && !parallel_ok(c) && g_tune.seq_first_stage >= 1 && !g_tune.mask_overlap &&
        !g_tune.ksplit) {
        int rc = step_pipelined(c, x, B, flags, target_wh, cls, loc, mask, box_out, refine_out, s);
        if (rc) return rc;
        c->track_B = B;
        return 0;
    }
    CHK(pipe_join(c, s, true));
    c->parity_now = c->last_parity = 0;
    int64_t pk, wi;
    memcpy(&pk, &c->penalty_k, 8); memcpy(&wi, &c->window_influence, 8);
    GraphKey key{3, B, flags, {x, target_wh, cls, loc, mask, box_out, refine_out, (const void *)pk, (const void *)wi}};
    StepRec rec = step_rec(c, refine_out);
    int rc = run_maybe_graph(c, key, s, rec, [&](hipStream_t st) {
        CHK(step_track_decode(c, rec, x, B, flags, target_wh, cls, loc, mask, box_out, refine_out, st, true, PH_ALL));
        return step_tail(c, rec, B, mask, box_out, refine_out, st);
    });
    if (rc) return rc;
    c->track_B = (flags & SMK_TRACK_MASK) ? B : 0;
    return 0;
}

int smk_set_pipeline(smk_ctx *c, int depth) {
    if (!c) return fail(SMK_E_ARG, "ctx is NULL");
    if (depth < 0 || depth > 2)
        return fail(SMK_E_ARG, "smk_set_pipeline: depth %d (0 = off, 1 = the tail beside the next frame's front end, 2 = its second part beside the next frame's heads)", depth);
    HIPCHK(hipSetDevice(c->device));
    CHK(pipe_quiesce(c));
    HIPCHK(hipDeviceSynchronize());
    c->tail_pending = false;
    if (depth > 0) {
        const char *hq = getenv("GPU_MAX_HW_QUEUES");
        if (hq && *hq && atoi(hq) < 2) {
            static bool said = false;
            if (!said) fprintf(stderr, "siammask_hip: GPU_MAX_HW_QUEUES=%s -- the pipelined frame step needs two hardware queues; running serial steps\n", hq);
            said = true;
            depth = 0;
        }
    }
    if (depth > 0) {
        if (!c->buf.count("p0#1")) {
            CHK(alloc_buf(c, "p0#1", c->buf_elems.at("p0")));
            CHK(alloc_buf(c, "p1#1", c->buf_elems.at("p1")));
            CHK(alloc_buf(c, "p2#1", c->buf_elems.at("p2")));
        }
        if (depth >= 2 && !c->buf.count("head0#1")) CHK(alloc_buf(c, "head0#1", c->buf_elems.at("head0")));
        if (c->ring_cursor) HIPCHK(hipMemcpy(c->ring_cursor + 2, c->ring_cursor, sizeof(int), hipMemcpyDeviceToDevice));
        if (!c->pipe_stream) {
            HIPCHK(hipStreamCreateWithFlags(&c->pipe_stream, hipStreamNonBlocking));
        }
        if (!c->pipe_cnt) HIPCHK(hipMalloc((void **)&c->pipe_cnt, 64));
        CHK(pipe_reset_counters(c));
        if (c->pipe_ev.empty()) {
            c->pipe_ev.resize(16);
            for (auto &e : c->pipe_ev) HIPCHK(hipEventCreateWithFlags(&e, hipEventDisableTiming));
        }
    }
    c->pipe_depth = depth;
    c->pipe_parity = 0;
    return 0;
}

int smk_pipeline_join(smk_ctx *c, void *stream) {
    if (!c) return fail(SMK_E_ARG, "ctx is NULL");
    HIPCHK(hipSetDevice(c->device));
    return pipe_join(c, (hipStream_t)stream, false);
}

int smk_pipeline_observe(smk_ctx *c, void *stream) {
    if (!c) return fail(SMK_E_ARG, "ctx is NULL");
    HIPCHK(hipSetDevice(c->device));
    if (!c->tail_pending) return 0;
    HIPCHK(hipStreamWaitEvent((hipStream_t)stream, c->tail_ev, 0));
    return 0;
}

int smk_set_result_ring(smk_ctx *c, double *box_ring, void *refine_ring_f16, int rows, int batch) {
    if (!c) return fail(SMK_E_ARG, "ctx is NULL");
    if (rows < 0 || (rows > 0 && !box_ring)) return fail(SMK_E_ARG, "smk_set_result_ring: rows %d / box ring %p", rows, (void *)box_ring);
    if (rows > 0 && (batch < 1 || batch > c->maxB)) return fail(SMK_E_ARG, "smk_set_result_ring: batch %d not in [1,%d]", batch, c->maxB);
    HIPCHK(hipSetDevice(c->device));
    CHK(pipe_quiesce(c));
    HIPCHK(hipDeviceSynchronize());
    c->tail_pending = false;
    for (auto &kv : c->graphs) hipGraphExecDestroy(kv.second);
    c->graphs.clear();
    c->graph_used.clear();
    c->graph_has_seq.clear();
    if (!c->ring_cursor) HIPCHK(hipMalloc((void **)&c->ring_cursor, 4 * sizeof(int)));
    HIPCHK(hipMemset(c->ring_cursor, 0, 4 * sizeof(int)));
    c->ring_box = rows ? box_ring : nullptr;
    c->ring_ref = rows ? refine_ring_f16 : nullptr;
    c->ring_rows = rows;
    c->ring_batch = rows ? batch : 0;
    return 0;
}

int smk_result_ring_cursor(smk_ctx *c, int *frames_out, int reset, void *stream) {
// ... 45 lines not shown
                    if (launch_cvt_out_x3(p, stream)) return fail(SMK_E_HIP, "cvt_out launch failed");
                }
                return 0;
            }
            CvtOutParams p{act(c, e.b, e.h, e.w, e.cs).p, dst, c->last_B, e.cn, e.h, e.w, e.cs, 0};
            if (launch_cvt_out(p, c->dtype, stream)) return fail(SMK_E_HIP, "cvt_out launch failed");
            return 0;
        }
    return fail(SMK_E_ARG, "smk_debug_read: unknown tensor %s", name);
}

struct TmpBufs {
    std::vector<void *> v;
    ~TmpBufs() { for (void *p : v) hipFree(p); }
    int alloc(void **p, size_t bytes) {
        HIPCHK(hipMalloc(p, bytes + 256));
        HIPCHK(hipMemset(*p, 0, bytes + 256));
        v.push_back(*p);
        return 0;
    }
};

static int fill_geom(const smk_conv_geom *g, PackedConv &pc, Act &in, ConvOpt &o, int &Ho, int &Wo) {
    const int cin_len = g->cin_len > 0 ? g->cin_len : g->Cin;
    pc.Ci = rup(cin_len, 8);
    pc.k = g->k;
    pc.K = g->k * g->k * pc.Ci;
    pc.Kpad = rup(pc.K, KPAD_ALIGN);
    pc.groups = 1;
    pc.N = g->Cout;
    pc.group_rows = pc.rows = rup(g->Cout, NPAD_ALIGN);
    in.H = g->H; in.W = g->W; in.C = rup(g->Cin, 8);
    o.stride = g->stride; o.pad = g->pad; o.dil = g->dil; o.relu = g->relu;
    o.cin_off = g->cin_off;
    o.win = g->win != 0; o.ups = g->ups != 0;
    o.Hl = g->Hl; o.Wl = g->Wl; o.org_y = g->org_y; o.org_x = g->org_x;
    o.pos_mul = g->pos_mul; o.pos_add = g->pos_add;
    const int Hl = (o.win || o.ups) ? g->Hl : g->H, Wl = (o.win || o.ups) ? g->Wl : g->W;
    Ho = (Hl + 2 * g->pad - g->dil * (g->k - 1) - 1) / g->stride + 1;
    Wo = (Wl + 2 * g->pad - g->dil * (g->k - 1) - 1) / g->stride + 1;
    if (Ho < 1 || Wo < 1) return fail(SMK_E_ARG, "conv geometry gives empty output");
    if (g->cin_off % 8 != 0) return fail(SMK_E_ARG, "cin_off must be a multiple of 8");
    if (g->cin_off + cin_len > g->Cin) return fail(SMK_E_ARG, "channel slice out of range");
    return 0;
}

static void pack_host(const smk_conv_geom *g, const PackedConv &pc, const float *w, const float *b,
                      std::vector<float> &rows, std::vector<float> &bias) {
    const int cin_len = g->cin_len > 0 ? g->cin_len : g->Cin;
    rows.assign((size_t)pc.rows * pc.Kpad, 0.f);
    bias.assign(pc.rows, 0.f);
    std::vector<double> one(g->Cout, 1.0);
    pack_rows(rows, 0, pc.Kpad, w, one.data(), g->Cout, cin_len, g->k, pc.Ci);
    if (b) for (int n = 0; n < g->Cout; ++n) bias[n] = b[n];
}

static int op_ks_scratch(ConvEnv &env) {
    static float *part[64] = {nullptr};
    static unsigned *cnt[64] = {nullptr};
    const int d = env.device;
    if (d < 0 || d >= 64) return 0;
    if (!part[d]) {
        HIPCHK(hipMalloc((void **)&part[d], KS_PART_FLOATS * sizeof(float)));
        HIPCHK(hipMalloc((void **)&cnt[d], KS_CNT * sizeof(unsigned)));
        HIPCHK(hipMemset(cnt[d], 0, KS_CNT * sizeof(unsigned)));
    }
    env.ks_part = part[d];
    env.ks_cnt = cnt[d];
    return 0;
}

static int plan_from_algo(int algo, const ConvParams &p, int dtype, ConvPlan &pl) {
    const int mode = algo & 0xff, code = (algo >> 8) & 0xff;
    switch (mode) {
    case 1: case 3: pl.kind = CK_NAIVE; return 0;
    case 4:
        pl.kind = CK_HALO; pl.halo_bm = (code & 15) == 1 ? 128 : 64;
        return conv_halo_eligible(p, dtype, pl.halo_bm) ? 0 : 1;
    case 5:
        pl.kind = CK_WREG; pl.wreg = code & 15; pl.stages = wreg_stages_from_code(code);
        if (pl.wreg < 1 || pl.wreg > 8) return -1;
        return conv_wreg_eligible(p, dtype) ? 0 : 1;
    case 6: pl.kind = CK_PP; return conv_pp_eligible(p, dtype) ? 0 : 1;
    default: pl.kind = CK_IGEMM; pl.tile = tile_from_code(code, p, dtype); return 0;
    }
}

int smk_op_conv2d_ex(int dtype, int algo, const smk_conv_geom *g, const float *x_dev, const float *w_host,
                     const float *b_host, const float *res_dev, const int32_t *pos_host, float *y_dev,
                     void *stream) {
    if (!g || !x_dev || !w_host || !y_dev) return fail(SMK_E_ARG, "smk_op_conv2d_ex: null argument");
    if (dtype != DT_F32 && dtype != DT_F16 && dtype != DT_F16X3) return fail(SMK_E_ARG, "bad dtype");
    const bool x3 = dtype == DT_F16X3;
    if (x3 && (((algo & 0xff) != 0 && (algo & 0xff) != 5) || g->cin_off || g->cin_len))
        return fail(SMK_E_ARG, "smk_op_conv2d_ex: split-operand convolutions: algo 0 (conv_igemm_kernel) or 5 (conv_wreg_kernel), no channel slice");
    const int ctx_dtype = dtype;
    dtype = kdtype(dtype);
    hipStream_t s = (hipStream_t)stream;
    PackedConv pc; Act in; ConvOpt o; int Ho, Wo;
    CHK(fill_geom(g, pc, in, o, Ho, Wo));
    std::vector<float> rows, bias;
    pack_host(g, pc, w_host, b_host, rows, bias);
    if (x3) {
        const int Ci0 = pc.Ci, K1 = pc.Kpad;
        pc.x3 = true;
        pc.alg_k = g->k * g->k * Ci0;
        pc.Ci = 3 * Ci0;
        pc.K = g->k * g->k * pc.Ci;
        pc.Kpad = rup(pc.K, KPAD_ALIGN);
        std::vector<float> osc;
        split_rows_x3(rows, pc.rows, K1, pc.Kpad, g->k * g->k, Ci0, osc);
        CHK(upload_oscale(pc, osc));
        in.C *= X3_PLANES;
    }
    std::vector<float> fused;
    if (x3 && g_tune.x3_fused && fuse_rows_x3(rows, pc, g->k * g->k, pc.Ci / 3, fused)) CHK(upload_packed(pc, rows, bias, dtype, &fused));
    else
    CHK(upload_packed(pc, rows, bias, dtype));
    TmpBufs tmp;
    tmp.v.push_back(pc.w); tmp.v.push_back(pc.bias);
    if (pc.w_frag) tmp.v.push_back(pc.w_frag);
    if (pc.w_frag16) tmp.v.push_back(pc.w_frag16);
    if (pc.oscale) tmp.v.push_back(pc.oscale);
    const size_t es = esize(dtype);
    CHK(tmp.alloc(&in.p, (size_t)g->B * g->H * g->W * in.C * es));
    CvtInParams ci{x_dev, in.p, g->B, g->Cin, g->H, g->W, x3 ? in.C / X3_PLANES : in.C, 0, x3 ? 1 : 0};
    if (x3 ? launch_cvt_in_x3(ci, s) : launch_cvt_in(ci, dtype, s)) return fail(SMK_E_HIP, "cvt_in launch failed");
    int *pos_dev = nullptr;
    if (pos_host) {
        CHK(tmp.alloc((void **)&pos_dev, sizeof(int) * 2 * g->B));
        HIPCHK(hipMemcpyAsync(pos_dev, pos_host, sizeof(int) * 2 * g->B, hipMemcpyHostToDevice, s));
        o.pos = pos_dev;
    }
    const int mode = algo & 0xff;
    const bool nchw = (mode == 2 || mode == 3);
    if (mode == 4) {
        CHK(upload_halo_pack(pc, rows, dtype));
        if (pc.w_frag_halo) tmp.v.push_back(pc.w_frag_halo);
        if (pc.w_halo) tmp.v.push_back(pc.w_halo);
    }
    Act out, res;
    out.H = Ho; out.W = Wo; out.C = rup(g->Cout, 8) * (x3 ? X3_PLANES : 1);
    if (res_dev && g->res_mode) {
        if (nchw) return fail(SMK_E_ARG, "residual is not supported with the NCHW epilogue");
        res = out;
        CHK(tmp.alloc(&res.p, (size_t)g->B * Ho * Wo * out.C * es));
        CvtInParams cr{res_dev, res.p, g->B, g->Cout, Ho, Wo, x3 ? out.C / X3_PLANES : out.C, 0, x3 ? 1 : 0};
        if (x3 ? launch_cvt_in_x3(cr, s) : launch_cvt_in(cr, dtype, s)) return fail(SMK_E_HIP, "cvt_in launch failed");
        o.res = &res; o.res_mode = g->res_mode;
    }
    ConvEnv env;
    env.dtype = ctx_dtype;
    HIPCHK(hipGetDevice(&env.device));
    CHK(op_ks_scratch(env));
    ConvParams p;
    if (nchw) {
        o.nchw_out = y_dev;
        CHK(conv_params(env, pc, in, nullptr, g->B, o, p));
    } else {
        CHK(tmp.alloc(&out.p, (size_t)g->B * Ho * Wo * out.C * es));
        CHK(conv_params(env, pc, in, &out, g->B, o, p));
    }
    ConvPlan pl;
    const int prc = plan_from_algo(algo, p, dtype, pl);
    if (prc < 0) return fail(SMK_E_ARG, "smk_op_conv2d_ex: wreg tile code 1..8");
    if (prc)
        return fail(SMK_E_ARG, "smk_op_conv2d_ex: %s", pl.kind == CK_HALO ? "geometry is not eligible for the halo kernel"
                    : (pl.kind == CK_WREG ? "geometry / dtype is not eligible for conv_wreg_kernel" : "geometry / dtype is not eligible for conv_pp_kernel"));
    ConvBatch cb;
    cb.n = 1;
    cb.p[0] = p;
    CHK(launch_plan(pl, cb, pc.w_halo, dtype, s, "conv"));
    if (!nchw) {
        CvtOutParams co{out.p, y_dev, g->B, g->Cout, Ho, Wo, out.C, 0, x3 ? out.C / X3_PLANES : 0};
        if (x3 ? launch_cvt_out_x3(co, s) : launch_cvt_out(co, dtype, s)) return fail(SMK_E_HIP, "cvt_out launch failed");
    }
    HIPCHK(hipStreamSynchronize(s));
    return 0;
}

static int seq_op_records(const smk_seq_op *ops, int n, const Act &xin, int device, const std::function<int(int, PackedConv &)> &pack,
                          const std::function<int(void **, size_t)> &alloc, std::vector<SeqRec> &rec, std::vector<Act> &outs) {
    const int dtype = DT_F16, B = ops[0].g.B;
    ConvEnv env;
    env.dtype = dtype;
    env.device = device;
    rec.assign(n, SeqRec());
    outs.assign(n, Act());
    for (int i = 0; i < n; ++i) {
        const smk_seq_op &op = ops[i];
        if (!op.w_host) return fail(SMK_E_ARG, "smk_op_conv_seq: layer %d has no weights", i);
        if (op.src >= i || op.res_src >= i) return fail(SMK_E_ARG, "smk_op_conv_seq: layer %d reads a later layer", i);
        if (op.g.B != B || op.g.win || op.g.ups) return fail(SMK_E_ARG, "smk_op_conv_seq: layer %d: one batch, no windows", i);
        const Act &in = op.src < 0 ? xin : outs[op.src];
        const int cin_have = op.src < 0 ? ops[0].g.Cin : ops[op.src].g.Cout;
        if (op.g.H != in.H || op.g.W != in.W || op.g.Cin != cin_have)
            return fail(SMK_E_ARG, "smk_op_conv_seq: layer %d geometry does not match its source", i);
        PackedConv pc; Act gin; ConvOpt o; int Ho, Wo;
        CHK(fill_geom(&op.g, pc, gin, o, Ho, Wo));
        CHK(pack(i, pc));
        outs[i].H = Ho; outs[i].W = Wo; outs[i].C = rup(op.g.Cout, 8);
        CHK(alloc(&outs[i].p, (size_t)B * Ho * Wo * outs[i].C * esize(dtype)));
        Act res;
        if (op.g.res_mode) {
            if (op.res_src < -1) return fail(SMK_E_ARG, "smk_op_conv_seq: layer %d wants a residual without a source", i);
            res = op.res_src < 0 ? xin : outs[op.res_src];
            if (res.H != Ho || res.W != Wo || res.C != outs[i].C)
                return fail(SMK_E_ARG, "smk_op_conv_seq: layer %d: residual shape differs from the output", i);
            o.res = &res; o.res_mode = op.g.res_mode;
        }
        ConvParams p;
        CHK(conv_params(env, pc, in, &outs[i], B, o, p));
        SeqLayer &L = rec[i].L;
        const int force_halo = op.cfg == SEQ_CFG_HALO128 ? 128 : (op.cfg == SEQ_CFG_HALO64 ? 64 : (op.cfg >= 0 ? -1 : 0));
        if (!seq_layer_from(p, dtype, L, force_halo)) return fail(SMK_E_ARG, "smk_op_conv_seq: layer %d cannot run inside a sequence%s", i, force_halo > 0 ? " on the patch-sharing tile" : "");
        if (op.cfg >= 0 && force_halo <= 0) {
#ifdef SMK_MEASURE
            if (op.cfg > 18) return fail(SMK_E_ARG, "smk_op_conv_seq: cfg 0..18");
#else
            if (op.cfg > 9 || (op.cfg >= 6 && op.cfg <= 8))
                return fail(SMK_E_ARG, "smk_op_conv_seq: cfg 0..5, 9 (6..8, 10..18 are measurement tiles: `make MEASURE=1`)");
#endif
            L.cfg = (signed char)op.cfg;
        }
        if (op.kstag >= 0) L.kstag = (signed char)(op.kstag != 0);
        L.sync = (signed char)(op.sync != 0);
        rec[i].wstd = pc.w_frag;
        rec[i].id = "op" + std::to_string(i);
    }
    return 0;
}

static SeqPlanStats plan_seq_ops(const smk_seq_op *ops, std::vector<SeqRec> &rec, const std::vector<Act> &outs, int grid) {
    std::vector<char> locked(rec.size());
    std::vector<const void *> read_after;
    for (size_t i = 0; i < rec.size(); ++i) {
        locked[i] = ops[i].cfg >= 0;
        if (ops[i].y_dev) read_after.push_back(outs[i].p);
    }
    return plan_seq(rec, {ops[0].g.B, grid >> 3, true}, locked.data(), read_after);
}

int smk_op_conv_seq(const smk_seq_op *ops, int n, const float *x_dev, int iters, float *usec_out, float *clk_us_out,
                    int *n_fused_out, void *stream) {
    if (!ops || !x_dev || n < 1 || n > SEQ_MAX || iters < 1) return fail(SMK_E_ARG, "smk_op_conv_seq: bad argument (1..%d layers)", SEQ_MAX);
    hipStream_t s = (hipStream_t)stream;
    const int dtype = DT_F16;
    const size_t es = esize(dtype);
    int dev = 0;
    HIPCHK(hipGetDevice(&dev));
    hipDeviceProp_t prop;
// ... 448 lines not shown
    PackedConv pc; Act in; ConvOpt o; int Ho, Wo;
    CHK(fill_geom(g, pc, in, o, Ho, Wo));
    std::vector<float> rows, bias;
    pack_host(g, pc, w, b, rows, bias);
    std::vector<float> xin((size_t)g->B * g->H * g->W * in.C, 0.f);
    for (int bb = 0; bb < g->B; ++bb)
        for (int c = 0; c < g->Cin; ++c)
            for (int yy = 0; yy < g->H; ++yy)
                for (int xx = 0; xx < g->W; ++xx)
                    xin[(((size_t)bb * g->H + yy) * g->W + xx) * in.C + c] =
                        x[(((size_t)bb * g->Cin + c) * g->H + yy) * g->W + xx];
    in.p = xin.data();
    pc.w = rows.data();
    pc.bias = bias.data();
    o.pos = pos;
    Act out;
    out.H = Ho; out.W = Wo; out.C = rup(g->Cout, 8);
    std::vector<float> obuf((size_t)g->B * Ho * Wo * out.C, 0.f);
    out.p = obuf.data();
    ConvEnv env;
    env.device = -1;
    ConvParams p;
    CHK(conv_params(env, pc, in, &out, g->B, o, p));
    for (int m = 0; m < p.M; ++m) {
        const RowInfo r = row_info(p, m, p.pos);
        for (int n = 0; n < g->Cout; ++n) {
            double acc = 0.0;
            for (int kvec = 0; kvec < p.K; kvec += 4) {
                const KDecode d = decode_k(kvec, p.Ci, p.kw);
                const long off = gather_offset(p, r, d, p.cin_off);
                if (off < 0) continue;
                for (int e = 0; e < 4; ++e) acc += (double)xin[off + e] * (double)rows[(size_t)n * p.Kpad + kvec + e];
            }
            double v = acc + bias[n];
            const int hw = Ho * Wo, bb = m / hw, ps = m - bb * hw;
            const double rv = (res && g->res_mode) ? res[((size_t)bb * g->Cout + n) * hw + ps] : 0.0;
            if (g->res_mode == RES_PRE_RELU) v += rv;
            if (g->relu) v = v > 0 ? v : 0;
            if (g->res_mode == RES_POST_RELU) v += rv;
            y[((size_t)bb * g->Cout + n) * hw + ps] = (float)v;
        }
    }
    return 0;
}

static void fake_pack(PackedConv &pc, int dtype) {
    static float dummy[64];
    pc.w = dummy; pc.bias = dummy;
    if (has_frag_pack(pc, dtype)) pc.w_frag = dummy;
    if (has_frag16_pack(pc, dtype)) pc.w_frag16 = dummy;
    if (has_halo_pack(pc, dtype)) pc.w_halo = dummy;
    if (has_frag_halo_pack(pc, dtype)) pc.w_frag_halo = dummy;
}

int smk_host_plan_conv(const smk_conv_geom *g, int dtype, int with_res, int *kernel, int *bm, int *bn, int *seq_cfg) {
    if (!g || !kernel || !bm || !bn || !seq_cfg) return fail(SMK_E_ARG, "smk_host_plan_conv: null argument");
    if (dtype != DT_F32 && dtype != DT_F16) return fail(SMK_E_ARG, "smk_host_plan_conv: dtype");
    PackedConv pc; Act in; ConvOpt o; int Ho, Wo;
    CHK(fill_geom(g, pc, in, o, Ho, Wo));
    static float dummy[64];
    in.p = dummy;
    fake_pack(pc, dtype);
    Act out, res;
    out.H = Ho; out.W = Wo; out.C = rup(g->Cout, 8); out.p = dummy;
    res = out;
    if (with_res) { o.res = &res; o.res_mode = RES_PRE_RELU; }
    ConvEnv env;
    env.device = -1;
    env.dtype = dtype;
    ConvParams p;
    CHK(conv_params(env, pc, in, &out, g->B, o, p));
    const ConvPlan pl = plan_conv(p, o, pc, dtype, g->B, MI355X_CUS);
    switch (pl.kind) {
    case CK_PP: *kernel = 3; *bm = 256; *bn = 256; break;
    case CK_WREG: *kernel = 2; *bm = WREG_TILE[pl.wreg][0]; *bn = WREG_TILE[pl.wreg][1]; break;
    case CK_HALO: *kernel = 1; *bm = pl.halo_bm; *bn = 128; break;
    default: *kernel = 0; *bm = pl.tile.bm; *bn = pl.tile.bn;
    }
    SeqLayer L;
    *seq_cfg = seq_layer_from(p, dtype, L) ? (int)L.cfg : -1;
    return 0;
}

int smk_host_plan_seq(const smk_seq_op *ops, int n, int grid, int *cfg, int *sync, int *a_stage) {
    if (!ops || n < 1 || n > 4 * SEQ_MAX || grid < 8 || grid % 8 || !cfg || !sync || !a_stage)
        return fail(SMK_E_ARG, "smk_host_plan_seq: bad argument (1..%d layers, a grid of whole teams)", 4 * SEQ_MAX);
    static char tensors[4 * SEQ_MAX + 1];
    Act xin;
    xin.H = ops[0].g.H; xin.W = ops[0].g.W; xin.C = rup(ops[0].g.Cin, 8); xin.p = tensors;
    int next = 1;
    std::vector<SeqRec> rec;
    std::vector<Act> outs;
    CHK(seq_op_records(ops, n, xin, -1, [](int, PackedConv &pc) { fake_pack(pc, DT_F16); return 0; },
                       [&](void **p, size_t) { *p = tensors + next++; return 0; }, rec, outs));
    plan_seq_ops(ops, rec, outs, grid);
    for (int i = 0; i < n; ++i) {
        cfg[i] = rec[i].L.cfg;
        sync[i] = rec[i].L.sync;
        a_stage[i] = rec[i].L.a_stage;
    }
    return 0;
}

}
```

siammask_amd/csrc/smk_kernels.h:

```cpp
#pragma once
#include <stdint.h>

#if defined(__HIPCC__)
#define SMK_HD __host__ __device__ inline
#else
#define SMK_HD inline
#endif

namespace smk {

enum { DT_F32 = 0, DT_F16 = 1, DT_F16X3 = 2 };
enum { RES_NONE = 0, RES_PRE_RELU = 1, RES_POST_RELU = 2 };
enum { OUT_NHWC = 0, OUT_NCHW_F32 = 1 };

constexpr int NPAD_ALIGN = 128;
constexpr int KPAD_ALIGN = 128;

struct ConvParams {
    const void *in;
    const void *wgt;
    const void *wgt_frag;
    const void *wgt_frag_halo;
    const float *bias;
    const void *res;
// ... 38 lines not shown
    int ksplit;
    float *ks_part;
    unsigned *ks_cnt;
    size_t ks_part_cap;
    int ks_cnt_cap;
};

constexpr int CONV_BATCH_MAX = 4;
struct ConvBatch {
    int n;
    int start[CONV_BATCH_MAX + 1];
    ConvParams p[CONV_BATCH_MAX];
};

struct SeqLayer {
    const void *in;
    const void *wgt_frag;
    const float *bias;
    const void *res;
    void *out;
    unsigned in_bytes, w_bytes;
    int kw_magic;
    unsigned short Hs, Ws, Hl, Wl, Ho, Wo, Cs, cin_off, Ci, Kpad, Nst, Cos, res_Cs, res_coff, cout_off, bar_ord;
    short org_y, org_x;
    signed char kh, kw, stride, stride_x, pad, dil, relu, res_mode, ci_shift;
    signed char cfg;
    signed char sync;
    signed char a_stage;
    signed char kstag;
    signed char res_nt;
    static constexpr const int *pos = nullptr;
    static constexpr int pos_mul = 0, pos_add = 0, ups = 0, g_cin_off = 0, g_wgt_off = 0, g_cout_off = 0;
    static constexpr int x3_out = 0, x3_res = 0, x3_in = 0, x3_ct = 0, x3_nreal = 0;
    static constexpr const float *oscale = nullptr;
};
static_assert(sizeof(SeqLayer) == 104, "SeqLayer packing");
constexpr int SEQ_CFG_C3C1_L3 = 20;
constexpr int SEQ_CFG_C3C1_L2 = 21;
constexpr int SEQ_CFG_C3C1_2ND = 22;
constexpr int SEQ_CFG_C3C1P_L3 = 26;
constexpr int SEQ_CFG_C3C1P_L2 = 27;
constexpr int SEQ_CFG_C2C3C1_L3 = 28;
constexpr int SEQ_CFG_C2C3C1_L2 = 29;
constexpr int SEQ_CFG_C2C3C1_MID = 30;
constexpr int SEQ_XCH_SLAB = 32768;
constexpr int SEQ_XCH_PAIRS = 16;
constexpr size_t SEQ_XCH_BYTES = (size_t)8 * SEQ_XCH_PAIRS * 4 * SEQ_XCH_SLAB;
constexpr int SEQ_CFG_HALO128 = 24;
constexpr int SEQ_CFG_HALO64 = 25;
constexpr int SEQ_YRES_IN = 2, SEQ_YRES_NOSTORE = 4, SEQ_LDS_HI = 8;
constexpr int SEQ_YRES_BYTES = 65536;
constexpr int SEQ_MAX = 36;
struct SeqArgs {
    int n, B;
    int flags, pad_;
    unsigned *bar;
    float *xch;
    int *err;
    int *err_host;
    unsigned long long *clk;
    unsigned long long *clk2;
    unsigned *exit_sem;
    SeqLayer L[SEQ_MAX];
};
static_assert(sizeof(SeqArgs) <= 4096, "the layer list travels in the kernel-argument segment");

struct Tuning {
    int xcd_mode = 1;
    int force_tile = 0;
    int min_blocks_x16 = 16;
    int stages = 0;
    int kt = 0;
    int prio = 0;
    int nt_store = 1;
    int halo = 1;
    int halo_db = 1;
    int chain = 1;
    int ksplit = 0;
    int xc_ch = 64;
    int l1_fused = 1;
    int stem_fused = 1;
    int xc_full = 0;
    int buf_lds = 1;
    int mask_overlap = 0;
    int chain_mask = 1;
    int nchw_tn_major = 1;
    int merge = 1;
    int merge_max_batch = 32;
    int rf_wreg = 3;
    int seq_fuse3 = 0;
    int seq_spoll = 1;
    int wreg = 1;
    int wreg_stages = 0;
    int seq = 1;
    int seq_min_batch = 5, seq_max_batch = 8;
    int seq_extra_batch = 12;
    int seq_mult_max = 24;
    int ablate = 0;
    int seq_tall = 2;
    int seq_kstag = 1;
    int res_nt = 1;
    int seq_fuse = 1;
    int rf_tile2 = 0;
    int pair_launch = 1;
    int corr_head = 1;
    int seq_yres = 1;
    int seq_search = 0;
    int seq_pair2d = 0;
    int seq_halo = 1;
    int seq_kstag_mask = 7;
    int seq_ds128 = 0;
    int seq_deep = 0;
    int seq_first_stage = 1;
    int wreg_policy = 1;
    int npw = 4;
    int a_stage = 0;
    int pp = 1;
    int main_prio = 3;
    int front_occ1 = 0;
    int wreg96 = 1;
    int x3_fused = 1;
    int wreg32 = 140;
    int pipe_late = 1;
};
extern Tuning g_tune;

struct KDecode { int kh_i, kw_i, c; };

SMK_HD KDecode decode_k(int kvec, int Ci, int kw) {
    KDecode d;
    int tap = kvec / Ci;
    d.c = kvec - tap * Ci;
    d.kh_i = tap / kw;
    d.kw_i = tap - d.kh_i * kw;
    return d;
}

struct RowInfo { int b, ly0, lx0, oy_org, ox_org; };

SMK_HD RowInfo row_info(const ConvParams &p, int m, const int *pos) {
    RowInfo r;
    int hw = p.Ho * p.Wo;
    r.b = m / hw;
    int rem = m - r.b * hw;
    int oy = rem / p.Wo;
    int ox = rem - oy * p.Wo;
    r.ly0 = oy * p.stride - p.pad;
    r.lx0 = ox * p.stride_x - p.pad;
    r.oy_org = p.org_y;
    r.ox_org = p.org_x;
    if (pos) {
        r.oy_org += pos[2 * r.b + 0] * p.pos_mul + p.pos_add;
        r.ox_org += pos[2 * r.b + 1] * p.pos_mul + p.pos_add;
    }
    return r;
}

SMK_HD long gather_offset(const ConvParams &p, const RowInfo &r, const KDecode &d, int cin_off) {
    int ly = r.ly0 + d.kh_i * p.dil;
    int lx = r.lx0 + d.kw_i * p.dil;
    if ((unsigned)ly >= (unsigned)p.Hl || (unsigned)lx >= (unsigned)p.Wl) return -1;
    int sy, sx;
    if (p.ups) {
        sy = (ly * p.Hs) / p.Hl;
        sx = (lx * p.Ws) / p.Wl;
    } else {
        sy = ly + r.oy_org;
        sx = lx + r.ox_org;
// ... 46 lines not shown
    const double *target_wh;
    const double *window;
    int *pos_out;
    double *box_out;
    double *part_val;
    int *part_idx;
    double *part_box;
    unsigned *arrived;
    int B, A, S, stride;
    float anchor_w[8], anchor_h[8];
    double penalty_k, window_influence;
    double *ring_box;
    int *ring_cursor;
    unsigned *ring_done;
    int ring_rows, ring_advance;
    int *ring_also;
    unsigned *mark, *mark_arrived;
};

struct RingParams {
    const double *box;
    const float *ref;
    double *box_ring;
    _Float16 *ref_ring;
    int *cursor;
    unsigned *done;
    int rows, B, n;
};

constexpr int CROP_MAX_B = 32;
struct CropParams {
    const unsigned char *frames;
    long frame_stride;
    float *out;
    int H, W, model_sz;
    int box[CROP_MAX_B][3];
    unsigned char avg[CROP_MAX_B][4];
};
struct PasteParams {
    const float *logits;
    unsigned char *mask_out;
    float *prob_out;
    int ms, W, H;
    float seg_thr, border;
    double inv_map[CROP_MAX_B][6];
};

struct TileChoice { int bm, bn, kt, stages; };
TileChoice choose_tile(const ConvParams &p, int dtype);
int launch_conv_mfma(const ConvParams &p, int dtype, TileChoice t, void *stream);
int launch_conv_mfma_batch(ConvBatch &cb, int dtype, TileChoice t, void *stream);
int launch_conv_naive(const ConvParams &p, int dtype, void *stream);
int conv_ksplit(const ConvParams &p, int dtype, const TileChoice &t);
__attribute__((visibility("hidden"))) bool conv_halo_eligible(const ConvParams &p, int dtype, int bm);
int launch_conv_halo(const ConvParams &p, int dtype, int bm, void *stream);
bool conv_wreg_eligible(const ConvParams &p, int dtype);
int launch_conv_wreg_batch(ConvBatch &cb, int bm, int bn, int stages, void *stream);
bool conv_pp_eligible(const ConvParams &p, int dtype);
int launch_conv_pp(const ConvParams &p, void *stream);
int launch_conv_seq(const SeqArgs &a, int grid, void *stream);
int launch_conv_pair(const SeqLayer &L3, const SeqLayer &L1, int code, int M, void *stream, int rows);
int conv_seq_occupancy();
int xcc_census(int grid, int *out_host);
struct RefineChainLayer {
    const void *w;
    const float *bias;
    int Kpad, Ci;
};
struct RefineChainParams {
    const void *d;
    const void *v2, *v1, *v0;
    int v2_cs, v1_cs, v0_cs;
    RefineChainLayer L[9];
    float *out;
    int B;
    unsigned long long *clk;
    _Float16 *ring;
    int *ring_cursor;
    unsigned *ring_done;
    int ring_rows;
    unsigned *tail_sem;
};
int launch_refine_chain(const RefineChainParams &p, void *stream);
int launch_chain_mask(const RefineChainParams &rp, ConvBatch &cb, void *stream);
int launch_xcorr(const XcorrParams &p, int dtype, void *stream);
int launch_xcorr_x3(const XcorrParams &p, void *stream);
void xcorr_prepare();
int launch_maxpool(const PoolParams &p, int dtype, void *stream);
int launch_stem_pool(const StemPoolParams &p, void *stream);
struct L1BlockParams {
    const void *x; void *y;
    const void *w1, *w2, *w3, *wd;
    const float *b1, *b2, *b3, *bd;
    int B, S, Cin, K1pad, K2pad, K3pad, Kdpad;
    unsigned long long *clk;
    int prio;
};
int launch_l1_block(const L1BlockParams &p, void *stream);
int launch_cvt_in(const CvtInParams &p, int dtype, void *stream);
int launch_cvt_out(const CvtOutParams &p, int dtype, void *stream);
int launch_cvt_in_x3(const CvtInParams &p, void *stream);
int launch_cvt_out_x3(const CvtOutParams &p, void *stream);
int launch_maxpool_x3(const PoolParams &p, void *stream);
int launch_decode(const DecodeParams &p, void *stream);
int launch_ring_commit(const RingParams &p, void *stream);
int launch_pipe_gate(unsigned *sem, int *err, int *err_host, void *stream, int long_wait = 0, unsigned *started_wait = nullptr, unsigned *started_set = nullptr);
int launch_pipe_done(unsigned *sem, void *stream);
int launch_crop_resize(const CropParams &p, int B, void *stream);
int launch_paste_mask(const PasteParams &p, int B, void *stream);
int launch_paste_labels(const PasteParams &p, int n_obj, void *stream);
struct RboxHdr {
    unsigned long long best;
    int ncomp, err;
};
struct RboxParams {
    const unsigned char *mask;
    int B, W, H, Wq, Wh;
    double min_area;
    RboxHdr *hdr; int *rows; unsigned long long *bits; int *parent;
    double *out;
};
int launch_mask_rbox(const RboxParams &p, void *stream);
const void *zero_page();

}
```

siammask_amd/ops.py:

```python
import ctypes

import numpy as np
import torch

from . import _lib

ALGO = {"mfma": 0, "naive": 1, "mfma_nchw": 2, "naive_nchw": 3, "halo": 4, "wreg": 5, "pp": 6}
WREG_TILE = {(64, 256): 1, (64, 128): 2, (64, 64): 3, (128, 256): 4, (128, 128): 5, (128, 64): 6, (96, 256): 7, (32, 64): 8}
TILE = {None: 0, "auto": 0, (128, 128): 1, (128, 64): 2, (64, 128): 3, (64, 64): 4, (256, 128): 5}


def _chk_cuda(*ts):
    for t in ts:
        if t is not None and not t.is_cuda:
            raise RuntimeError("siammask_amd.ops run on the MI355X only (got a CPU tensor)")


def tile_code(tile=None, kt=0, stages=0):
    return TILE[tile] | ({0: 0, 128: 1, 256: 2}[kt] << 4) | ({0: 0, 2: 1, 3: 2, 4: 3}[stages] << 6)


def wreg_code(tile, stages=0):
    return WREG_TILE[tuple(tile)] | ({0: 0, 8: 1, 3: 2, 4: 3}[stages] << 6)


def conv2d(x, w, b=None, stride=1, pad=0, dil=1, relu=False, res=None, res_mode=1, dtype="f32",
           algo="mfma", tile=None, win=None, ups=None, pos=None, pos_mul=0, pos_add=0, org=(0, 0),
           cin_off=0, cin_len=0, kt=0, stages=0):
    _chk_cuda(x, res)
    x = x.contiguous().float()
    B, Cin, H, W = x.shape
    w = np.ascontiguousarray(w.detach().cpu().numpy() if isinstance(w, torch.Tensor) else w, dtype=np.float32)
    bb = None if b is None else np.ascontiguousarray(
        b.detach().cpu().numpy() if isinstance(b, torch.Tensor) else b, dtype=np.float32)
    g = _lib.ConvGeom()
    g.B, g.Cin, g.H, g.W = B, Cin, H, W
    g.Cout, g.k, g.stride, g.pad, g.dil = w.shape[0], w.shape[2], stride, pad, dil
    g.relu = int(bool(relu))
    g.res_mode = res_mode if res is not None else 0
    g.cin_off, g.cin_len = cin_off, cin_len
    g.org_y, g.org_x = org
    g.pos_mul, g.pos_add = pos_mul, pos_add
    Hl, Wl = H, W
    if win is not None:
        g.win, g.Hl, g.Wl = 1, win[0], win[1]
        Hl, Wl = win
    if ups is not None:
        g.ups, g.Hl, g.Wl = 1, ups[0], ups[1]
        Hl, Wl = ups
    Ho = (Hl + 2 * pad - dil * (g.k - 1) - 1) // stride + 1
    Wo = (Wl + 2 * pad - dil * (g.k - 1) - 1) // stride + 1
    y = torch.empty((B, g.Cout, Ho, Wo), dtype=torch.float32, device=x.device)
    p = None if pos is None else np.ascontiguousarray(pos, dtype=np.int32)
    r = None if res is None else res.contiguous().float()
    code = ALGO[algo] | ((wreg_code(tile, stages) if algo == "wreg" else tile_code(tile, kt, stages)) << 8)
    vp = lambda a: a.ctypes.data_as(ctypes.c_void_p) if a is not None else None
    with torch.cuda.device(x.device):
        _lib.check(_lib.lib().smk_op_conv2d_ex(
            _lib.DTYPE[dtype], code, ctypes.byref(g), x.data_ptr(), vp(w), vp(bb),
            r.data_ptr() if r is not None else None, vp(p), y.data_ptr(), _lib.current_stream_ptr()))
    return y


SEQ_CFG = {None: -1, (64, 256): 0, (64, 128): 1, (64, 64): 2, (128, 256): 3, (128, 128): 4, "deep": 5,
           "no_a": 6, "no_w": 7, "no_mfma": 8, (128, 64): 9,
           "abl10": 10, "abl11": 11, "abl12": 12, "abl13": 13, "abl14": 14, "old64x128": 15, "old128x256": 16, "old64x256": 17, "old64x64": 18,
           "halo128": 24, "halo64": 25}


def seq_ops(x_shape, layers):
    B = x_shape[0]
    arr = (_lib.SeqOp * len(layers))()
    keep = []
    shapes = [tuple(x_shape[1:])]
    for i, l in enumerate(layers):
        w = np.ascontiguousarray(l["w"], dtype=np.float32)
        b = None if l.get("b") is None else np.ascontiguousarray(l["b"], dtype=np.float32)
        keep += [w, b]
        src = l.get("src", i - 1)
        cin, H, W = shapes[src + 1]
        k, stride, pad, dil = w.shape[2], l.get("stride", 1), l.get("pad", 0), l.get("dil", 1)
        g = arr[i].g
        g.B, g.Cin, g.H, g.W = B, cin, H, W
        g.Cout, g.k, g.stride, g.pad, g.dil = w.shape[0], k, stride, pad, dil
        g.relu = int(bool(l.get("relu", False)))
        g.res_mode = l.get("res_mode", 1) if "res" in l else 0
        Ho = (H + 2 * pad - dil * (k - 1) - 1) // stride + 1
        Wo = (W + 2 * pad - dil * (k - 1) - 1) // stride + 1
        shapes.append((w.shape[0], Ho, Wo))
        arr[i].src = src
        arr[i].res_src = l.get("res", -2)
        arr[i].sync = int(bool(l.get("sync", True)))
        arr[i].cfg = SEQ_CFG[l.get("tile")]
        arr[i].kstag = l.get("kstag", -1)
        arr[i].w_host = w.ctypes.data
        arr[i].b_host = b.ctypes.data if b is not None else None
    return arr, keep, shapes[1:]


def _wanted(want_outputs, i):
    return want_outputs is True or (want_outputs not in (False, None) and i in want_outputs)


def conv_seq(x, layers, iters=1, want_outputs=True, info=None):
    _chk_cuda(x)
    x = x.contiguous().float()
    B = x.shape[0]
    n = len(layers)
    arr, keep, shapes = seq_ops(x.shape, layers)
    outs = []
    for i, shape in enumerate(shapes):
        if _wanted(want_outputs, i):
            y = torch.empty((B,) + shape, dtype=torch.float32, device=x.device)
            outs.append(y)
            arr[i].y_dev = y.data_ptr()
        elif want_outputs not in (True, False, None):
            outs.append(None)
    us = ctypes.c_float(0.0)
    clk = np.zeros(2 * n, dtype=np.float32)
    nfused = ctypes.c_int(0)
    with torch.cuda.device(x.device):
        _lib.check(_lib.lib().smk_op_conv_seq(arr, n, x.data_ptr(), iters, ctypes.byref(us),
                                              clk.ctypes.data_as(ctypes.c_void_p), ctypes.byref(nfused), _lib.current_stream_ptr()))
    if info is not None:
        info["fused_pairs"] = nfused.value
    return outs, us.value, clk.reshape(n, 2)


def plan_seq(x_shape, layers, want_outputs=True, grid=256):
    arr, keep, _ = seq_ops(x_shape, layers)
    n = len(layers)
    for i in range(n):
        if _wanted(want_outputs, i):
            arr[i].y_dev = 1
    out = [(ctypes.c_int * n)() for _ in range(3)]
# ... 47 lines not shown
```

Baseline: 14250.

## Add specialized mask-head slab kernel and drop side-stream mask overlap

Adds a dedicated kernel for the 1x1 mask3 conv (K=256, 625 positions, 32-channel slabs). Each workgroup keeps a slab's weights in registers, double-buffers the activation loads through swizzled LDS, and runs 32x32x16 MFMAs. The output is staged in LDS so the NCHW f32 result can be written with aligned vector stores. The kernel is wired into the fused refine-chain+mask launch and into the conv planner, and is on by default. The old side-stream mask overlap path is removed, which adds a specialized code path with strict eligibility checks.

```diff
diff --git a/siammask_amd/_lib.py b/siammask_amd/_lib.py
--- a/siammask_amd/_lib.py
+++ b/siammask_amd/_lib.py
@@ -20,7 +20,7 @@
     "smk_op_maxpool3x3s2", "smk_op_conv_seq", "smk_host_conv2d_ex", "smk_host_plan_conv", "smk_host_plan_seq", "smk_bench_conv", "smk_packed_size", "smk_export_packed",
     "smk_import_packed", "smk_crop_resize", "smk_paste_mask", "smk_paste_labels", "smk_mask_rbox_workspace", "smk_mask_rbox",
     "smk_trk_state_bytes", "smk_trk_set", "smk_trk_plan", "smk_trk_advance", "smk_crop_resize_dev", "smk_paste_mask_dev",
-    "smk_host_trk_plan", "smk_host_trk_advance",
+    "smk_host_trk_plan", "smk_host_trk_advance", "smk_host_mask_slabs",
 )
 
 
@@ -126,6 +126,7 @@
     L.smk_paste_mask_dev.argtypes = [fp, fp, ci, ci, vp, ci, ci, ci, ci, ctypes.c_float, ctypes.c_float, vp, fp, vp]
     L.smk_op_conv_seq.argtypes = [ctypes.POINTER(SeqOp), ci, fp, ci, ctypes.POINTER(ctypes.c_float), fp, ip, vp]
     L.smk_host_plan_seq.argtypes = [ctypes.POINTER(SeqOp), ci, ci, ip, ip, ip]
+    L.smk_host_mask_slabs.argtypes = [ctypes.c_uint64, ci, ci, ctypes.POINTER(ctypes.c_longlong), ci, ip]
     L.smk_bench_conv.argtypes = [ci, ci, gp, ci, ci, ctypes.POINTER(ctypes.c_float), vp]
     for name in SYMBOLS:
         fn = getattr(L, name)
diff --git a/siammask_amd/csrc/conv_igemm.hip b/siammask_amd/csrc/conv_igemm.hip
--- a/siammask_amd/csrc/conv_igemm.hip
+++ b/siammask_amd/csrc/conv_igemm.hip
@@ -866,19 +866,11 @@
 }
 namespace smk {
 #include "refine_chain_body.inc"
+#include "mask_head_body.inc"
 constexpr int CM_CONV_LDS = IgemmLds<2, 2, 1, 128, 2>::v;
-constexpr int CM_LDS = CMax<RC_LDS, 2 * CM_CONV_LDS>::v;
-
-__global__ __launch_bounds__(1024) void chain_mask_kernel(const RefineChainParams rp, const ConvBatch cb) {
-    __shared__ __attribute__((aligned(16))) unsigned char smem[CM_LDS];
-    if ((int)blockIdx.x < rp.B) {
-        refine_chain_body<false>(rp, (int)blockIdx.x, smem);
-    } else {
-        const int half = threadIdx.x >> 9;
-        const int bx = 2 * ((int)blockIdx.x - rp.B) + half;
-        if (bx < cb.start[cb.n])
-            conv_igemm_body<_Float16, 2, 2, 1, 128, OUT_NCHW_F32, 2>(cb, bx, 0, half * 512, smem + half * CM_CONV_LDS);
-    }
+constexpr int CM_LDS = CMax<CMax<RC_LDS, 2 * CM_CONV_LDS>::v, MS_LDS>::v;
+
+__device__ __forceinline__ void chain_mask_done(const RefineChainParams &rp) {
     if (rp.tail_sem) {
         __syncthreads();
         if (threadIdx.x == 0) {
@@ -891,16 +883,37 @@
     }
 }
 
-int launch_chain_mask(const RefineChainParams &rp, ConvBatch &cb, void *stream) {
+__global__ __launch_bounds__(1024) void chain_mask_kernel(const RefineChainParams rp, const ConvBatch cb, const int slab) {
+    __shared__ __attribute__((aligned(16))) unsigned char smem[CM_LDS];
+    if ((int)blockIdx.x < rp.B) {
+        refine_chain_body<false>(rp, (int)blockIdx.x, smem);
+    } else if (slab) {
+        mask_slab_body(mask_slab_params(cb.p[0]), (int)blockIdx.x - rp.B, (int)gridDim.x - rp.B, smem);
+    } else {
+        const int half = threadIdx.x >> 9;
+        const int bx = 2 * ((int)blockIdx.x - rp.B) + half;
+        if (bx < cb.start[cb.n])
+            conv_igemm_body<_Float16, 2, 2, 1, 128, OUT_NCHW_F32, 2>(cb, bx, 0, half * 512, smem + half * CM_CONV_LDS);
+    }
+    chain_mask_done(rp);
+}
+
+int launch_chain_mask(const RefineChainParams &rp, ConvBatch &cb, int slab, void *stream) {
     if (rp.v2_cs != 32 || rp.v1_cs != 16 || rp.v0_cs != 8 || cb.n != 1) return -1;
     ConvParams &p = cb.p[0];
     if (p.out_mode != OUT_NCHW_F32 || p.groups > 1) return -1;
+    if (slab) {
+        if (!mask_slab_launchable(p) || rp.B != p.B || rp.B >= 256) return -1;
+        const int grid = mask_slab_grid(p.B, p.N, 256 - rp.B);
+        hipLaunchKernelGGL(chain_mask_kernel, dim3(rp.B + grid), dim3(1024), 0, (hipStream_t)stream, rp, cb, 1);
+        return hipGetLastError() == hipSuccess ? 0 : -4;
+    }
     const int tiles = ((p.M + 127) / 128) * ((p.Nst + 127) / 128);
     if (tiles & 1) return 1;
     cb.start[0] = 0;
     for (int i = 1; i <= CONV_BATCH_MAX; ++i) cb.start[i] = tiles;
     p.ksplit = 1;
-    hipLaunchKernelGGL(chain_mask_kernel, dim3(rp.B + (tiles + 1) / 2), dim3(1024), 0, (hipStream_t)stream, rp, cb);
+    hipLaunchKernelGGL(chain_mask_kernel, dim3(rp.B + (tiles + 1) / 2), dim3(1024), 0, (hipStream_t)stream, rp, cb, 0);
     return hipGetLastError() == hipSuccess ? 0 : -4;
 }
 
diff --git a/siammask_amd/csrc/conv_plan.cpp b/siammask_amd/csrc/conv_plan.cpp
--- a/siammask_amd/csrc/conv_plan.cpp
+++ b/siammask_amd/csrc/conv_plan.cpp
@@ -358,11 +358,16 @@
     return g_tune.pp == 2 || K >= 2304;
 }
 
+bool mask_slab_choice(const ConvParams &p, const ConvOpt &o, int dtype) {
+    return g_tune.mask_slab && !o.algo_naive && !o.halo && !o.wreg && !o.tile_code && mask_slab_eligible(p, dtype);
+}
+
 ConvPlan plan_conv(const ConvParams &p, const ConvOpt &o, const PackedConv &pc, int dtype, int B, long ncu) {
     const int kd = kdtype(dtype);
     ConvPlan pl;
     pl.tile = tile_from_code(o.tile_code, p, kd);
     if (o.algo_naive) { pl.kind = CK_NAIVE; return pl; }
+    if (mask_slab_choice(p, o, kd)) { pl.kind = CK_MASK_SLAB; return pl; }
     int bm = halo_choice(pc, p, o, kd);
     if (bm && !o.halo && conv_ksplit(p, kd, pl.tile) > 1) bm = 0;
     if (pp_choice(p, o, kd, ncu)) { pl.kind = CK_PP; return pl; }
@@ -396,6 +401,7 @@
     switch (pl.kind) {
     case CK_NAIVE: return "conv_naive";
     case CK_PP: return "conv_pp<f16,256x256>";
+    case CK_MASK_SLAB: return "mask_slab<f16,32x625>";
     case CK_HALO: snprintf(kn, sizeof(kn), "conv3x3_halo<%s,%dx128>", dt, pl.halo_bm); break;
     case CK_WREG: snprintf(kn, sizeof(kn), "conv_wreg<%s,%dx%d,s%d%s>", dt, WREG_TILE[pl.wreg][0], WREG_TILE[pl.wreg][1], pl.stages, mg); break;
     default:
diff --git a/siammask_amd/csrc/conv_plan.h b/siammask_amd/csrc/conv_plan.h
--- a/siammask_amd/csrc/conv_plan.h
+++ b/siammask_amd/csrc/conv_plan.h
@@ -55,7 +55,7 @@
 
 #pragma GCC visibility push(hidden)
 
-enum ConvKernel { CK_NAIVE, CK_IGEMM, CK_HALO, CK_WREG, CK_PP };
+enum ConvKernel { CK_NAIVE, CK_IGEMM, CK_HALO, CK_WREG, CK_PP, CK_MASK_SLAB };
 struct ConvPlan {
     int kind = CK_IGEMM;
     smk::TileChoice tile{};
@@ -72,6 +72,7 @@
 int wreg_stages(int ctx_dtype, int B);
 int wreg_stages_from_code(int code);
 bool pp_choice(const smk::ConvParams &p, const ConvOpt &o, int dtype, long ncu);
+bool mask_slab_choice(const smk::ConvParams &p, const ConvOpt &o, int dtype);
 
 ConvPlan plan_conv(const smk::ConvParams &p, const ConvOpt &o, const PackedConv &pc, int dtype, int B, long ncu);
 ConvPlan plan_conv_batch(const smk::ConvBatch &cb, const ConvOpt *const *o, int lead, int dtype, int B, long ncu);
diff --git a/siammask_amd/csrc/engine.cpp b/siammask_amd/csrc/engine.cpp
--- a/siammask_amd/csrc/engine.cpp
+++ b/siammask_amd/csrc/engine.cpp
@@ -277,9 +277,9 @@
     bool done_folded = false;
     bool ring_ref_folded = false;
     bool has_seq = false;
-    bool mask_join_pending = false;
     struct DeferredMask {
         bool have = false;
+        bool slab = false;
         ConvParams p = {};
         double flop = 0.0, bytes = 0.0;
     } deferred_mask;
@@ -923,6 +923,7 @@
         break;
     }
     case CK_NAIVE: rc = launch_conv_naive(cb.p[0], dtype, s); break;
+    case CK_MASK_SLAB: rc = launch_mask_slab(cb.p[0], 0, s); break;
     default: rc = launch_conv_mfma_batch(cb, dtype, pl.tile, s);
     }
     if (rc == 1) return fail(SMK_E_STATE, "internal: %s is not eligible for the kernel planned for it", what);
@@ -1226,7 +1227,7 @@
 }
 
 static int seq_track(smk_ctx *c, StepRec &rec, const float *x, int B, int flags, float *cls, float *loc, float *mask,
-                     hipStream_t s, bool defer_mask_join = false, int phase = PH_ALL) {
+                     hipStream_t s, int phase = PH_ALL) {
     auto X = [c](int C) { return c->dtype == DT_F16X3 ? X3_PLANES * C : C; };
     const bool x3 = c->dtype == DT_F16X3;
     const int nbt = nbranch(c);
@@ -1296,11 +1297,8 @@
             const ConvParams &mp = rec.deferred_mask.p;
             rec.deferred_mask.flop = 2.0 * mp.M * (double)mp.N * mp.kh * mp.kw * mp.Ci;
             rec.deferred_mask.bytes = (double)mp.M * mp.Ci * esize(c->dtype) + (double)mp.M * mp.N * 4 + (double)mp.N * mp.Ci * esize(c->dtype);
+            rec.deferred_mask.slab = plan_conv(mp, om, it->second, c->dtype, B, c->ncu).kind == CK_MASK_SLAB;
             rec.deferred_mask.have = true;
-        } else if (defer_mask_join && !par && !c->prof && g_tune.mask_overlap && c->side[0]) {
-            CHK(stream_dep(c, s, c->side[0]));
-            CHK(run_conv(c, "mask3", h0, nullptr, B, om, c->side[0]));
-            rec.mask_join_pending = true;
         } else {
             CHK(run_conv(c, "mask3", h0, nullptr, B, om, s));
         }
@@ -1406,7 +1404,7 @@
             cb.p[0] = rec.deferred_mask.p;
             ProfScope ps(c, s, "refine_chain+mask3", "chain_mask", flop + rec.deferred_mask.flop, cbytes + rec.deferred_mask.bytes);
             if (rec.tail_fold) rp.tail_sem = c->pipe_cnt;
-            const int rc = launch_chain_mask(rp, cb, s);
+            const int rc = launch_chain_mask(rp, cb, rec.deferred_mask.slab ? 1 : 0, s);
             rp.tail_sem = nullptr;
             if (rc == 0) {
                 rec.deferred_mask.have = false;
@@ -1919,6 +1917,7 @@
     {"nchw_tn_major", &g_tune.nchw_tn_major, "*", KNOB_BOOL, nullptr},
     {"chain", &g_tune.chain, "*", KNOB_BOOL, nullptr},
     {"chain_mask", &g_tune.chain_mask, "*", KNOB_BOOL, nullptr},
+    {"mask_slab", &g_tune.mask_slab, "*", KNOB_BOOL, nullptr},
     {"corr_head", &g_tune.corr_head, "*", KNOB_BOOL, nullptr},
     {"pair_launch", &g_tune.pair_launch, "0..3", KNOB_RAW, nullptr},
     {"halo", &g_tune.halo, "0|1|64|128", KNOB_RAW, nullptr},
@@ -1930,7 +1929,6 @@
     {"l1_fused", &g_tune.l1_fused, "*", KNOB_BOOL, nullptr},
     {"buf_lds", &g_tune.buf_lds, "*", KNOB_BOOL, nullptr},
     {"a_stage", &g_tune.a_stage, "*", KNOB_BOOL, nullptr},
-    {"mask_overlap", &g_tune.mask_overlap, "*", KNOB_BOOL, nullptr},
     {"wreg", &g_tune.wreg, "0..7", KNOB_RAW, nullptr},
     {"wreg_policy", &g_tune.wreg_policy, "0|1", KNOB_RAW, nullptr},
     {"wreg_stages", &g_tune.wreg_stages, "0|3..8", KNOB_RAW, "0|3|4"},
@@ -2128,12 +2126,12 @@
 }
 
 static int step_track_decode(smk_ctx *c, StepRec &rec, const float *x, int B, int flags, const double *target_wh, float *cls, float *loc,
-                             float *mask, double *box_out, float *refine_out, hipStream_t st, bool defer_mask_join, int phase) {
+                             float *mask, double *box_out, float *refine_out, hipStream_t st, int phase) {
     rec.defer_mask = refine_out && mask && (flags & SMK_TRACK_MASK) && !(flags & SMK_TRACK_NO_MASK_HEAD) &&
                      kdtype(c->dtype) == DT_F16 && g_tune.chain && g_tune.chain_mask && !parallel_ok(c) &&
                      (B <= 16 ||
                       rec.two);
-    CHK(seq_track(c, rec, x, B, flags, cls, loc, mask, st, defer_mask_join, phase));
+    CHK(seq_track(c, rec, x, B, flags, cls, loc, mask, st, phase));
     return seq_decode(c, rec, cls, loc, B, target_wh, c->pos_dev, box_out, st);
 }
 
@@ -2148,7 +2146,6 @@
     if (refine_out) CHK(seq_refine(c, rec, B, refine_out, st, part));
     if (part == 1) return 0;
     if (rec.deferred_mask.have) CHK(mask3());
-    if (rec.mask_join_pending) CHK(stream_dep(c, c->side[0], st));
     if (c->ring_rows > 0 && refine_out && c->ring_ref && !rec.ring_ref_folded) {
         RingParams rg{box_out, refine_out, nullptr, (_Float16 *)c->ring_ref, c->ring_cursor,
                       (unsigned *)(c->ring_cursor + 1), c->ring_rows, B, 127 * 127};
@@ -2181,7 +2178,7 @@
         rec.mark_fold = true;
         rec.two = two;
         rec.seq_exit = two;
-        CHK(step_track_decode(c, rec, x, B, flags, target_wh, cls, loc, mask, box_out, refine_out, st, false, PH_BACK));
+        CHK(step_track_decode(c, rec, x, B, flags, target_wh, cls, loc, mask, box_out, refine_out, st, PH_BACK));
         if (two && !rec.seq_exit_done && launch_pipe_done(c->pipe_cnt + 7, st)) return fail(SMK_E_HIP, "pipe_done launch failed");
         return 0;
     };
@@ -2262,7 +2259,7 @@
     HIPCHK(hipSetDevice(c->device));
     CHK(seq_health(c));
     hipStream_t s = (hipStream_t)stream;
-    if (c->pipe_depth > 0 && refine_out && !c->prof && !parallel_ok(c) && g_tune.seq_first_stage >= 1 && !g_tune.mask_overlap &&
+    if (c->pipe_depth > 0 && refine_out && !c->prof && !parallel_ok(c) && g_tune.seq_first_stage >= 1 &&
         !g_tune.ksplit) {
         int rc = step_pipelined(c, x, B, flags, target_wh, cls, loc, mask, box_out, refine_out, s);
         if (rc) return rc;
@@ -2276,7 +2273,7 @@
     GraphKey key{3, B, flags, {x, target_wh, cls, loc, mask, box_out, refine_out, (const void *)pk, (const void *)wi}};
     StepRec rec = step_rec(c, refine_out);
     int rc = run_maybe_graph(c, key, s, rec, [&](hipStream_t st) {
-        CHK(step_track_decode(c, rec, x, B, flags, target_wh, cls, loc, mask, box_out, refine_out, st, true, PH_ALL));
+        CHK(step_track_decode(c, rec, x, B, flags, target_wh, cls, loc, mask, box_out, refine_out, st, PH_ALL));
         return step_tail(c, rec, B, mask, box_out, refine_out, st);
     });
     if (rc) return rc;
@@ -2488,6 +2485,7 @@
         if (pl.wreg < 1 || pl.wreg > 8) return -1;
         return conv_wreg_eligible(p, dtype) ? 0 : 1;
     case 6: pl.kind = CK_PP; return conv_pp_eligible(p, dtype) ? 0 : 1;
+    case 7: pl.kind = CK_MASK_SLAB; return mask_slab_eligible(p, dtype) ? 0 : 1;
     default: pl.kind = CK_IGEMM; pl.tile = tile_from_code(code, p, dtype); return 0;
     }
 }
@@ -2539,7 +2537,7 @@
         o.pos = pos_dev;
     }
     const int mode = algo & 0xff;
-    const bool nchw = (mode == 2 || mode == 3);
+    const bool nchw = (mode == 2 || mode == 3 || mode == 7);
     if (mode == 4) {
         CHK(upload_halo_pack(pc, rows, dtype));
         if (pc.w_frag_halo) tmp.v.push_back(pc.w_frag_halo);
@@ -2572,7 +2570,8 @@
     if (prc < 0) return fail(SMK_E_ARG, "smk_op_conv2d_ex: wreg tile code 1..8");
     if (prc)
         return fail(SMK_E_ARG, "smk_op_conv2d_ex: %s", pl.kind == CK_HALO ? "geometry is not eligible for the halo kernel"
-                    : (pl.kind == CK_WREG ? "geometry / dtype is not eligible for conv_wreg_kernel" : "geometry / dtype is not eligible for conv_pp_kernel"));
+                    : (pl.kind == CK_WREG ? "geometry / dtype is not eligible for conv_wreg_kernel"
+                    : (pl.kind == CK_MASK_SLAB ? "geometry / dtype is not eligible for mask_slab_kernel" : "geometry / dtype is not eligible for conv_pp_kernel")));
     ConvBatch cb;
     cb.n = 1;
     cb.p[0] = p;
@@ -3187,6 +3186,19 @@
     return 0;
 }
 
+int smk_host_mask_slabs(unsigned long long out_addr, int B, int N, long long *rows, int cap, int *n_out) {
+    if (!rows || !n_out || B < 1 || N < 1) return fail(SMK_E_ARG, "smk_host_mask_slabs: bad argument");
+    const int n = mask_slab_count(B, N);
+    *n_out = n;
+    if (cap < n) return fail(SMK_E_ARG, "smk_host_mask_slabs: %d slabs, room for %d", n, cap);
+    for (int s = 0; s < n; ++s) {
+        const MaskSlabSplit sp = mask_slab_split(out_addr, B, N, s);
+        long long *r = rows + 6 * (size_t)s;
+        r[0] = sp.g0; r[1] = sp.len; r[2] = sp.sh; r[3] = sp.head; r[4] = sp.nvec; r[5] = sp.tail;
+    }
+    return 0;
+}
+
 int smk_host_plan_seq(const smk_seq_op *ops, int n, int grid, int *cfg, int *sync, int *a_stage) {
     if (!ops || n < 1 || n > 4 * SEQ_MAX || grid < 8 || grid % 8 || !cfg || !sync || !a_stage)
         return fail(SMK_E_ARG, "smk_host_plan_seq: bad argument (1..%d layers, a grid of whole teams)", 4 * SEQ_MAX);
diff --git a/siammask_amd/csrc/mask_head.hip b/siammask_amd/csrc/mask_head.hip
--- /dev/null
+++ b/siammask_amd/csrc/mask_head.hip
@@ -0,0 +1,41 @@
+#include <hip/hip_runtime.h>
+#include "smk_kernels.h"
+
+namespace smk {
+#include "mask_head_body.inc"
+
+__global__ __launch_bounds__(MS_THREADS) void mask_slab_kernel(const MaskSlabParams p) {
+    __shared__ __attribute__((aligned(16))) unsigned char smem[MS_LDS];
+    mask_slab_body(p, (int)blockIdx.x, (int)gridDim.x, smem);
+}
+
+bool mask_slab_eligible(const ConvParams &p, int dtype) {
+    if (dtype != DT_F16 || p.out_mode != OUT_NCHW_F32 || !p.wgt_frag) return false;
+    if (p.kh != 1 || p.kw != 1 || p.stride != 1 || p.stride_x != 1 || p.pad != 0 || p.ups || p.pos || p.org_y || p.org_x) return false;
+    if (p.Ci != MS_K || p.K != MS_K || p.Kpad != MS_K || p.x3_in || p.x3_ct || p.oscale) return false;
+    if (p.Hl != p.Hs || p.Wl != p.Ws || p.Ho * p.Wo != MS_HW || p.Hs * p.Ws != MS_HW || p.M != p.B * MS_HW) return false;
+    if (p.groups > 1 || p.relu || p.res || p.res_mode != RES_NONE || p.B < 1 || p.N < 1) return false;
+    if (p.Cs % 8 || p.cin_off % 8 || p.cin_off + MS_K > p.Cs) return false;
+    const long rows = (long)((p.N + MS_NB - 1) / MS_NB) * MS_NB;
+    return p.w_bytes != 0 && (long)p.w_bytes >= rows * MS_K * 2 && (long)p.in_bytes >= (long)p.B * MS_HW * p.Cs * 2 && p.in_bytes < 0x7fff0000u;
+}
+
+bool mask_slab_launchable(const ConvParams &p) {
+    return mask_slab_eligible(p, DT_F16) && p.in && p.out && p.bias && !((uintptr_t)p.in & 15) && !((uintptr_t)p.out & 3);
+}
+
+int mask_slab_grid(int B, int N, int ncu) {
+    const int nslab = mask_slab_count(B, N);
+    int g = ncu;
+    if (B < g) g -= g % B;
+    return g < nslab ? g : nslab;
+}
+
+int launch_mask_slab(const ConvParams &p, int grid, void *stream) {
+    if (!mask_slab_launchable(p)) return 1;
+    if (grid <= 0) grid = mask_slab_grid(p.B, p.N, 256);
+    hipLaunchKernelGGL(mask_slab_kernel, dim3(grid), dim3(MS_THREADS), 0, (hipStream_t)stream, mask_slab_params(p));
+    return hipGetLastError() == hipSuccess ? 0 : -4;
+}
+
+}
diff --git a/siammask_amd/csrc/mask_head_body.inc b/siammask_amd/csrc/mask_head_body.inc
--- /dev/null
+++ b/siammask_amd/csrc/mask_head_body.inc
@@ -0,0 +1,124 @@
+
+typedef _Float16 ms_half8 __attribute__((ext_vector_type(8)));
+typedef float ms_floatx16 __attribute__((ext_vector_type(16)));
+typedef float ms_floatx4 __attribute__((ext_vector_type(4)));
+typedef unsigned ms_uint4 __attribute__((ext_vector_type(4)));
+
+constexpr int MS_THREADS = 1024;
+constexpr int MS_PASS_BLKS = 5, MS_NPASS = 4;
+constexpr int MS_ROW = MS_K * 2;
+constexpr int MS_IMG_BYTES = (MS_NB * MS_HW + 4) * 4;
+constexpr int MS_STAGE_BYTES = MS_PASS_BLKS * 32 * MS_ROW;
+constexpr int MS_LDS = MS_IMG_BYTES + MS_STAGE_BYTES + MS_NB * 4;
+static_assert(MS_PASS_BLKS * MS_NPASS * 32 >= MS_HW && MS_IMG_BYTES % 16 == 0 && MS_LDS <= 160 * 1024, "mask slab LDS layout");
+static_assert(MS_PASS_BLKS * 32 * (MS_ROW / 16) == 5 * MS_THREADS, "five staging loads per thread and pass");
+
+__device__ __forceinline__ void mask_slab_body(const MaskSlabParams &p, int wg, int nwg, unsigned char *smem) {
+    float *img = (float *)smem;
+    unsigned char *stage = smem + MS_IMG_BYTES;
+    float *bias_s = (float *)(smem + MS_IMG_BYTES + MS_STAGE_BYTES);
+    const int tid = threadIdx.x, lane = tid & 63;
+    const int wave = __builtin_amdgcn_readfirstlane(tid >> 6);
+    const int fm = lane & 31, fh = lane >> 5;
+    const bool mul = wave < MS_PASS_BLKS;
+    const int nslab = mask_slab_count(p.B, p.N);
+    constexpr int KS = MS_K / 16;
+
+    const __amdgpu_buffer_rsrc_t rs_a = __builtin_amdgcn_make_buffer_rsrc((void *)p.in, 0, p.in_bytes, 0x00020000);
+    const __amdgpu_buffer_rsrc_t rs_w = __builtin_amdgcn_make_buffer_rsrc((void *)p.w_frag, 0, p.w_bytes, 0x00020000);
+    const int row_bytes = p.Cs * 2;
+    const int a_thread = (tid >> 5) * row_bytes + p.cin_off * 2 + (tid & 31) * 16;
+    ms_uint4 pre[5];
+    auto fetch = [&](int b, int pass) {
+        const int pos0 = pass * (MS_PASS_BLKS * 32);
+        const int base = (b * MS_HW + pos0) * row_bytes + a_thread;
+#pragma unroll
+        for (int i = 0; i < 5; ++i) {
+            const int ok = -(int)(pos0 + i * 32 + (tid >> 5) < MS_HW);
+            pre[i] = __builtin_amdgcn_raw_buffer_load_b128(rs_a, ((base + i * 32 * row_bytes) & ok) | (0x7ffff000 & ~ok), 0, 0);
+        }
+    };
+    ms_half8 wf[KS];
+    auto load_w = [&](int blk) {
+#pragma unroll
+        for (int k = 0; k < KS; ++k)
+            wf[k] = __builtin_bit_cast(ms_half8, __builtin_amdgcn_raw_buffer_load_b128(rs_w, ((blk * KS + k) * 64 + lane) * 16, 0, 0));
+    };
+
+    int s = wg;
+    if (s < nslab) {
+        fetch(s % p.B, 0);
+        if (mul) load_w(s / p.B);
+    }
+    for (; s < nslab; s += nwg) {
+        const int b = s % p.B, blk = s / p.B;
+        const int sn = s + nwg;
+        const MaskSlabSplit sp = mask_slab_split((unsigned long long)(uintptr_t)p.out, p.B, p.N, s);
+        if (tid < MS_NB) bias_s[tid] = p.bias[blk * MS_NB + tid];
+#pragma unroll 1
+        for (int pass = 0; pass < MS_NPASS; ++pass) {
+#pragma unroll
+            for (int i = 0; i < 5; ++i) {
+                const int g = i * MS_THREADS + tid, r = g >> 5, c = g & 31;
+                *(ms_uint4 *)(stage + r * MS_ROW + ((c ^ (r & 31)) << 4)) = pre[i];
+            }
+            __syncthreads();
+            if (pass + 1 < MS_NPASS) fetch(b, pass + 1);
+            else if (sn < nslab) fetch(sn % p.B, 0);
+            if (mul) {
+                ms_floatx16 acc;
+#pragma unroll
+                for (int r = 0; r < 16; ++r) acc[r] = 0.f;
+                const int row = 32 * wave + fm;
+                const unsigned char *arow = stage + row * MS_ROW;
+                int sw = (row & 31) ^ fh;
+                asm volatile("" : "+v"(sw));
+#pragma unroll
+                for (int k4 = 0; k4 < KS; k4 += 4) {
+                    ms_half8 a[4];
+#pragma unroll
+                    for (int q = 0; q < 4; ++q) a[q] = *(const ms_half8 *)(arow + (((2 * (k4 + q)) ^ sw) << 4));
+#pragma unroll
+                    for (int q = 0; q < 4; ++q) acc = __builtin_amdgcn_mfma_f32_32x32x16_f16(wf[k4 + q], a[q], acc, 0, 0, 0);
+                    __builtin_amdgcn_sched_barrier(0);
+                }
+                if (pass + 1 == MS_NPASS && sn < nslab && sn / p.B != blk) load_w(sn / p.B);
+                const int pos = (pass * MS_PASS_BLKS + wave) * 32 + fm;
+                if (pos < MS_HW) {
+                    float *o = img + sp.sh + pos + 4 * fh * MS_HW;
+                    const ms_floatx4 *bq = (const ms_floatx4 *)(bias_s + 4 * fh);
+#pragma unroll
+                    for (int q = 0; q < 4; ++q) {
+                        const ms_floatx4 bv = bq[2 * q];
+#pragma unroll
+                        for (int e = 0; e < 4; ++e) o[(8 * q + e) * MS_HW] = acc[4 * q + e] + bv[e];
+                    }
+                }
+            }
+            __syncthreads();
+        }
+        float *og = p.out + sp.g0;
+        const float *iv = img + sp.sh + sp.head;
+        float *ov = og + sp.head;
+        constexpr int NV = (MS_NB * MS_HW / 4 + MS_THREADS - 1) / MS_THREADS;
+        ms_floatx4 x[NV];
+#pragma unroll
+        for (int j = 0; j < NV; ++j) {
+            const int v = j * MS_THREADS + tid;
+            x[j] = *(const ms_floatx4 *)(iv + 4 * v);
+        }
+#pragma unroll
+        for (int j = 0; j < NV; ++j) {
+            const int v = j * MS_THREADS + tid;
+            if (v < sp.nvec) {
+                if (p.nt_store) __builtin_nontemporal_store(x[j], (ms_floatx4 *)(ov + 4 * v));
+                else *(ms_floatx4 *)(ov + 4 * v) = x[j];
+            }
+        }
+        if (tid < sp.head) og[tid] = img[sp.sh + tid];
+        if (tid >= 64 && tid - 64 < sp.tail) {
+            const int i = sp.head + 4 * sp.nvec + tid - 64;
+            og[i] = img[sp.sh + i];
+        }
+    }
+}
diff --git a/siammask_amd/csrc/smk_kernels.h b/siammask_amd/csrc/smk_kernels.h
--- a/siammask_amd/csrc/smk_kernels.h
+++ b/siammask_amd/csrc/smk_kernels.h
@@ -144,8 +144,8 @@
     int stem_fused = 1;
     int xc_full = 0;
     int buf_lds = 1;
-    int mask_overlap = 0;
     int chain_mask = 1;
+    int mask_slab = 1;
     int nchw_tn_major = 1;
     int merge = 1;
     int merge_max_batch = 32;
@@ -358,7 +358,41 @@
     unsigned *tail_sem;
 };
 int launch_refine_chain(const RefineChainParams &p, void *stream);
-int launch_chain_mask(const RefineChainParams &rp, ConvBatch &cb, void *stream);
+int launch_chain_mask(const RefineChainParams &rp, ConvBatch &cb, int slab, void *stream);
+constexpr int MS_NB = 32;
+constexpr int MS_HW = 625;
+constexpr int MS_K = 256;
+struct MaskSlabParams {
+    const void *in;
+    const void *w_frag;
+    const float *bias;
+    float *out;
+    int B, N, Cs, cin_off;
+    unsigned in_bytes, w_bytes;
+    int nt_store;
+};
+SMK_HD int mask_slab_count(int B, int N) { return B * ((N + MS_NB - 1) / MS_NB); }
+struct MaskSlabSplit { long long g0; int len, sh, head, nvec, tail; };
+SMK_HD MaskSlabSplit mask_slab_split(unsigned long long out_addr, int B, int N, int s) {
+    MaskSlabSplit r;
+    const int b = s % B, n0 = (s / B) * MS_NB;
+    const int nch = N - n0 < MS_NB ? N - n0 : MS_NB;
+    r.g0 = ((long long)b * N + n0) * MS_HW;
+    r.len = nch * MS_HW;
+    r.sh = (int)(((out_addr >> 2) + (unsigned long long)r.g0) & 3);
+    r.head = (4 - r.sh) & 3;
+    r.nvec = (r.len - r.head) >> 2;
+    r.tail = r.len - r.head - 4 * r.nvec;
+    return r;
+}
+bool mask_slab_eligible(const ConvParams &p, int dtype);
+bool mask_slab_launchable(const ConvParams &p);
+SMK_HD MaskSlabParams mask_slab_params(const ConvParams &p) {
+    return MaskSlabParams{p.in, p.wgt_frag, p.bias, (float *)p.out, p.B, p.N, p.Cs, p.cin_off, p.in_bytes, p.w_bytes, p.nt_store};
+}
+int mask_slab_grid(int B, int N, int ncu);
+int launch_mask_slab(const ConvParams &p, int grid, void *stream);
+
 int launch_xcorr(const XcorrParams &p, int dtype, void *stream);
 int launch_xcorr_x3(const XcorrParams &p, void *stream);
 void xcorr_prepare();
diff --git a/siammask_amd/ops.py b/siammask_amd/ops.py
--- a/siammask_amd/ops.py
+++ b/siammask_amd/ops.py
@@ -5,7 +5,7 @@
 
 from . import _lib
 
-ALGO = {"mfma": 0, "naive": 1, "mfma_nchw": 2, "naive_nchw": 3, "halo": 4, "wreg": 5, "pp": 6}
+ALGO = {"mfma": 0, "naive": 1, "mfma_nchw": 2, "naive_nchw": 3, "halo": 4, "wreg": 5, "pp": 6, "mask_slab": 7}
 WREG_TILE = {(64, 256): 1, (64, 128): 2, (64, 64): 3, (128, 256): 4, (128, 128): 5, (128, 64): 6, (96, 256): 7, (32, 64): 8}
 TILE = {None: 0, "auto": 0, (128, 128): 1, (128, 64): 2, (64, 128): 3, (64, 64): 4, (256, 128): 5}
 
@@ -26,8 +26,8 @@
 
 def conv2d(x, w, b=None, stride=1, pad=0, dil=1, relu=False, res=None, res_mode=1, dtype="f32",
            algo="mfma", tile=None, win=None, ups=None, pos=None, pos_mul=0, pos_add=0, org=(0, 0),
-           cin_off=0, cin_len=0, kt=0, stages=0):
-    _chk_cuda(x, res)
+           cin_off=0, cin_len=0, kt=0, stages=0, out=None):
+    _chk_cuda(x, res, out)
     x = x.contiguous().float()
     B, Cin, H, W = x.shape
     w = np.ascontiguousarray(w.detach().cpu().numpy() if isinstance(w, torch.Tensor) else w, dtype=np.float32)
@@ -50,7 +50,12 @@
         Hl, Wl = ups
     Ho = (Hl + 2 * pad - dil * (g.k - 1) - 1) // stride + 1
     Wo = (Wl + 2 * pad - dil * (g.k - 1) - 1) // stride + 1
-    y = torch.empty((B, g.Cout, Ho, Wo), dtype=torch.float32, device=x.device)
+    if out is None:
+        y = torch.empty((B, g.Cout, Ho, Wo), dtype=torch.float32, device=x.device)
+    else:
+        if out.dtype != torch.float32 or not out.is_contiguous() or out.numel() != B * g.Cout * Ho * Wo:
+            raise ValueError("out: contiguous float32, %d elements" % (B * g.Cout * Ho * Wo))
+        y = out.view(B, g.Cout, Ho, Wo)
     p = None if pos is None else np.ascontiguousarray(pos, dtype=np.int32)
     r = None if res is None else res.contiguous().float()
     code = ALGO[algo] | ((wreg_code(tile, stages) if algo == "wreg" else tile_code(tile, kt, stages)) << 8)
```

After: 13440. 5.7% lower.
